# barlettacarmen/CrCNN

Measured on AMD Instinct MI355X. Metric: encrypted images/sec, higher is better.
Workload: dtype u64

## Files before the change

crcnn_amd/binding.py:

```python
import ctypes
import os
import re

import numpy as np

_HERE = os.path.dirname(os.path.abspath(__file__))
LIB_PATH = os.path.join(_HERE, "lib", "libcrcnn_hip.so")
HEADER = os.path.join(os.path.dirname(_HERE), "include", "crcnn_hip.h")

u64 = ctypes.c_uint64
PU = ctypes.POINTER(u64)
VP = ctypes.c_void_p
CI = ctypes.c_int
SZ = ctypes.c_size_t

COEFF, NTT, NTTP, NTTL, NTTL1, NTTLC, NTTLS = 0, 1, 2, 3, 4, 5, 6


class CrcError(RuntimeError):
    def __init__(self, status, what=""):
        self.status = status
        super().__init__(f"{what}: {_strerror(status)} (status {status}, hip error {_lib.crc_last_hip_error() if _lib else '?'})")


# ... 78 lines not shown
    L.crc_square_relin.argtypes = [VP, VP, SZ, VP, CI, VP, VP, VP]
    L.crc_square_relin_forms.argtypes = [VP, VP, CI, SZ, VP, CI, VP, CI, VP, VP]
    L.crc_square_pool_relin_supported.argtypes = [VP, CI, CI, CI]
    L.crc_square_pool_relin_work_bytes.restype = SZ; L.crc_square_pool_relin_work_bytes.argtypes = [VP] + [CI] * 9
    L.crc_square_pool_relin_forms.argtypes = [VP, VP, CI] + [CI] * 8 + [VP, CI, VP, VP, CI, VP, VP]
    L.crc_poly2_relin_work_bytes.restype = SZ; L.crc_poly2_relin_work_bytes.argtypes = [VP, SZ, CI]
    L.crc_poly2_relin_forms.argtypes = [VP, VP, CI, SZ, VP, CI, VP, VP, VP, VP, CI, VP, VP]
    L.crc_multiply_relin_work_bytes.restype = SZ; L.crc_multiply_relin_work_bytes.argtypes = [VP, SZ, CI]
    L.crc_multiply.argtypes = [VP, VP, VP, SZ, VP, VP, VP]
    L.crc_multiply_relin_forms.argtypes = [VP, VP, VP, CI, SZ, VP, CI, VP, CI, VP, VP]
    L.crc_poly3_relin_work_bytes.restype = SZ; L.crc_poly3_relin_work_bytes.argtypes = [VP, SZ, CI]
    L.crc_poly3_relin_forms.argtypes = [VP, VP, CI, SZ, VP, CI, VP, VP, VP, VP, VP, CI, VP, VP]
    L.crc_poly2_pool_relin_supported.argtypes = [VP, CI, CI, CI]
    L.crc_poly2_pool_relin_work_bytes.restype = SZ; L.crc_poly2_pool_relin_work_bytes.argtypes = [VP] + [CI] * 9
    L.crc_poly2_pool_relin_forms.argtypes = [VP, VP, CI] + [CI] * 8 + [VP, CI, VP, VP, VP, VP, CI, VP, VP]
    L.crc_conv2d_forms.argtypes = [VP, VP, VP, CI, VP] + [CI] * 9 + [CI, CI, VP, VP, VP]
    L.crc_dense_forms.argtypes = [VP, VP, VP, CI, VP, CI, CI, CI, CI, CI, VP, VP, VP]
    L.crc_pack28.argtypes = [VP, VP, SZ, CI, VP]
    L.crc_limb_supported.argtypes = [VP, CI, CI, CI]
    L.crc_limb_tensor_bytes.restype = SZ; L.crc_limb_tensor_bytes.argtypes = [VP, CI, CI, CI, CI]
    L.crc_limb_weights_bytes.restype = SZ; L.crc_limb_weights_bytes.argtypes = [VP, CI, CI, CI, CI]
    L.crc_limb_pack_weights.argtypes = [VP, VP, CI, CI, CI, CI, VP, VP]
    L.crc_limb_pack_weights_tile.argtypes = [VP, VP, CI, CI, CI, CI, CI, CI, VP, VP]
    L.crc_limb_pack_tensor_at.argtypes = [VP, VP, CI, CI, CI, CI, CI, VP, CI, CI, VP]
    L.crc_plan_mac.argtypes = [VP] + [CI] * 10 + [ctypes.POINTER(CI)]
    L.crc_plan_mac_scalar.argtypes = [VP] + [CI] * 9 + [ctypes.POINTER(CI)]
    L.crc_scalar_weights_bytes.restype = SZ; L.crc_scalar_weights_bytes.argtypes = [VP, CI, CI, CI, CI]
    L.crc_scalar_supported.argtypes = [VP] + [CI] * 9
    L.crc_scalar_pack_weights.argtypes = [VP, VP, CI, CI, CI, CI, CI, VP, ctypes.POINTER(CI), VP]
    L.crc_plan_fold_pool.argtypes = [VP] + [CI] * 12 + [ctypes.POINTER(CI)]
    L.crc_plan_hoist_pool.argtypes = [VP] + [CI] * 22 + [ctypes.POINTER(CI)]
    L.crc_limb_pack_tensor.argtypes = [VP, VP, CI, CI, CI, CI, CI, VP, VP]
    L.crc_limb_conv1_supported.argtypes = [VP] + [CI] * 8
    L.crc_limb_conv1_weights_bytes.restype = SZ; L.crc_limb_conv1_weights_bytes.argtypes = [VP]
    L.crc_limb_conv1_pack_weights.argtypes = [VP, VP, CI, CI, CI, VP, VP]
    L.crc_limb_conv1_weights_bytes_for.restype = SZ; L.crc_limb_conv1_weights_bytes_for.argtypes = [VP, CI, CI, CI]
    L.crc_limb_conv1_form.argtypes = [VP] + [CI] * 8
    L.crc_conv2d_forms_work_bytes.restype = SZ; L.crc_conv2d_forms_work_bytes.argtypes = [VP] + [CI] * 12
    L.crc_square.argtypes = [VP, VP, SZ, VP, VP, VP]
    L.crc_relinearize.argtypes = [VP, VP, SZ, VP, CI, VP, VP, VP]
    L.crc_import_seal.argtypes = [VP, PU, CI, PU]
    L.crc_export_seal.argtypes = [VP, PU, CI, PU]
    L.crc_params_hash.argtypes = [VP, PU]
    for f_ in ("ct", "evk", "pk", "sk"):
        getattr(L, f"crc_seal_{f_}_bytes").restype = SZ
    L.crc_seal_ct_bytes.argtypes = [VP, CI]; L.crc_seal_evk_bytes.argtypes = [VP, CI]; L.crc_seal_pk_bytes.argtypes = [VP]; L.crc_seal_sk_bytes.argtypes = [VP]
    L.crc_seal_ct_save.argtypes = [VP, PU, CI, VP, SZ, ctypes.POINTER(SZ)]
    L.crc_seal_ct_load.argtypes = [VP, VP, SZ, PU, CI, ctypes.POINTER(CI), ctypes.POINTER(SZ)]
    L.crc_seal_evk_save.argtypes = [VP, PU, CI, VP, SZ, ctypes.POINTER(SZ)]
    L.crc_seal_evk_load.argtypes = [VP, VP, SZ, PU, ctypes.POINTER(CI)]
    L.crc_seal_pk_save.argtypes = [VP, PU, VP, SZ, ctypes.POINTER(SZ)]
    L.crc_seal_pk_load.argtypes = [VP, VP, SZ, PU]
    L.crc_seal_sk_save.argtypes = [VP, PU, VP, SZ, ctypes.POINTER(SZ)]
    L.crc_seal_sk_load.argtypes = [VP, VP, SZ, PU]
    L.crc_h5_dataset_count.argtypes = [ctypes.c_char_p, ctypes.c_char_p, ctypes.POINTER(SZ)]
    L.crc_h5_read_f32.argtypes = [ctypes.c_char_p, ctypes.c_char_p, ctypes.POINTER(ctypes.c_float), SZ, ctypes.POINTER(SZ)]
    L.crc_h5_list.argtypes = [ctypes.c_char_p, ctypes.c_char_p, SZ]
    L.crc_keygen.argtypes = [VP, u64, PU, PU]
    L.crc_gen_evk.argtypes = [VP, u64, PU, CI, PU]
    L.crc_encrypt.argtypes = [VP, PU, PU, SZ, u64, PU]
    L.crc_encrypt_dev_work_bytes.restype = SZ; L.crc_encrypt_dev_work_bytes.argtypes = [VP, SZ]
    L.crc_encrypt_dev.argtypes = [VP, VP, VP, SZ, u64, VP, VP, VP]
    PB = ctypes.POINTER(ctypes.c_uint8)
    L.crc_random_key.argtypes = [PB]
    L.crc_chacha20_block.argtypes = [PB, ctypes.c_uint32, PB, PB]
    L.crc_keygen_key.argtypes = [VP, PB, PU, PU]
# ... 415 lines not shown
                                   self.p(d_y), self.p(d_work), self.stream), "crc_conv2d")
        else:
            _chk(self.L.crc_conv2d_forms(self.c, self.p(d_x), self.p(d_w), w_form, self.p(d_bias), B, zd, xd, yd, xs, ys, xf, yf, nf, in_form, out_form,
                                         self.p(d_y), self.p(d_work), self.stream), "crc_conv2d_forms")

    def limb_supported(self, zd, xf=1, yf=1):
        return bool(self.L.crc_limb_supported(self.c, zd, xf, yf))

    def limb_tensor_bytes(self, B, zd, xd=1, yd=1):
        return self.L.crc_limb_tensor_bytes(self.c, B, zd, xd, yd)

    def limb_weights_bytes(self, nf, zd, xf=1, yf=1):
        return self.L.crc_limb_weights_bytes(self.c, nf, zd, xf, yf)

    def limb_pack_weights(self, d_w_ntt, nf, zd, xf, yf, d_wl):
        _chk(self.L.crc_limb_pack_weights(self.c, self.p(d_w_ntt), nf, zd, xf, yf, self.p(d_wl), self.stream), "crc_limb_pack_weights")

    def plan_mac(self, zd, xd, yd, xs, ys, xf, yf, nf, B, matrix_cores=True):
        wf = CI(0)
        _chk(self.L.crc_plan_mac(self.c, zd, xd, yd, xs, ys, xf, yf, nf, int(B or 0), 1 if matrix_cores else 0, ctypes.byref(wf)), "crc_plan_mac")
        return wf.value

    def plan_fold_pool(self, zd, xd, yd, xs, ys, xf, yf, nf, pxs, pys, pxf, pyf):
        f = CI(0)
        _chk(self.L.crc_plan_fold_pool(self.c, zd, xd, yd, xs, ys, xf, yf, nf, pxs, pys, pxf, pyf, ctypes.byref(f)), "crc_plan_fold_pool")
        return bool(f.value)

    def plan_hoist_pool(self, up, conv, pool, B, matrix_cores=True):
        h = CI(0)
        _chk(self.L.crc_plan_hoist_pool(self.c, *(tuple(up) if up else (0,) * 8), *conv, *pool, int(B or 0), 1 if matrix_cores else 0, ctypes.byref(h)),
             "crc_plan_hoist_pool")
        return bool(h.value)

    def scalar_weights_bytes(self, nf, zd, xf=1, yf=1):
        return self.L.crc_scalar_weights_bytes(self.c, nf, zd, xf, yf)

    def scalar_supported(self, B, zd, xd, yd, xs, ys, xf, yf, nf):
        return bool(self.L.crc_scalar_supported(self.c, B, zd, xd, yd, xs, ys, xf, yf, nf))

    def scalar_pack_weights(self, d_w, w_stride, nf, zd, xf, yf, d_ws):
        const = CI(1)
        rc = self.L.crc_scalar_pack_weights(self.c, self.p(d_w), w_stride, nf, zd, xf, yf, self.p(d_ws), ctypes.byref(const), self.stream)
        if rc == -1 and const.value == 0:
            return False
        _chk(rc, "crc_scalar_pack_weights")
        return True

    def plan_mac_scalar(self, zd, xd, yd, xs, ys, xf, yf, nf, B):
        wf = CI(0)
        _chk(self.L.crc_plan_mac_scalar(self.c, zd, xd, yd, xs, ys, xf, yf, nf, int(B or 0), ctypes.byref(wf)), "crc_plan_mac_scalar")
        return wf.value

    def limb_pack_weights_tile(self, d_w_tile, nf, f0, ft, zd, xf, yf, d_wl):
        _chk(self.L.crc_limb_pack_weights_tile(self.c, self.p(d_w_tile), nf, f0, ft, zd, xf, yf, self.p(d_wl), self.stream), "crc_limb_pack_weights_tile")

    def limb_pack_tensor(self, d_x, in_form, B, zd, xd, yd, d_xl):
        _chk(self.L.crc_limb_pack_tensor(self.c, self.p(d_x), in_form, B, zd, xd, yd, self.p(d_xl), self.stream), "crc_limb_pack_tensor")

    def limb_pack_tensor_at(self, d_x, in_form, B, zd, xd, yd, d_xl, Btot, b0):
        _chk(self.L.crc_limb_pack_tensor_at(self.c, self.p(d_x), in_form, B, zd, xd, yd, self.p(d_xl), Btot, b0, self.stream), "crc_limb_pack_tensor_at")

    def limb_conv1_supported(self, zd, xd, yd, xs, ys, xf, yf, nf):
        return bool(self.L.crc_limb_conv1_supported(self.c, zd, xd, yd, xs, ys, xf, yf, nf))

    def limb_conv1_weights_bytes(self):
        return self.L.crc_limb_conv1_weights_bytes(self.c)
# ... 300 lines not shown
```

crcnn_amd/csrc/abi.hip:

```cpp
#include <cstdlib>
#include <cstring>
#include "kernels.h"
#include "chacha.h"
#include "work_arena.h"

#define CHECK_CTX(c) do { if (!(c) || (c)->device < 0) return CRC_ERR_INVALID_ARGUMENT; \
        int dev_ = -1; if (hipGetDevice(&dev_) != hipSuccess || dev_ != (c)->device) HIPCHK(hipSetDevice((c)->device)); } while (0)
#define RUN(x) do { int rc_ = (x); if (rc_) return rc_; } while (0)
static inline hipStream_t S(void *s) { return (hipStream_t)s; }
static inline bool form_ok(int f) { return f == CRC_COEFF || f == CRC_NTT; }
static inline bool nform_ok(int f) { return f == CRC_COEFF || f == CRC_NTT || f == CRC_NTTP; }
static inline bool lform_ok(int f) { return nform_ok(f) || f == CRC_NTTL; }
static inline bool limb_in(int f) { return f == CRC_NTTL || f == CRC_NTTLS; }
static inline u64 *work_base(void *d_work) { return WorkArena(d_work).take<u64>(0); }
static inline size_t work_bytes(size_t words) { WorkArena a; a.take<u64>(words); return a.bytes(); }

extern "C" int crc_plain_to_ntt(crc_ctx *c, const uint64_t *d_plain, size_t count, uint64_t *d_out, void *stream)
{
    CHECK_CTX(c); if (!d_plain || !d_out) return CRC_ERR_INVALID_ARGUMENT;
    return k_plain_ntt(c, d_plain, count, 1, true, d_out, S(stream));
}
extern "C" int crc_plain_expand(crc_ctx *c, const uint64_t *d_compact, size_t count, uint64_t *d_plain, void *stream)
{
    CHECK_CTX(c); if (!d_compact || !d_plain) return CRC_ERR_INVALID_ARGUMENT;
// ... 101 lines not shown
    if (!crc_limb_supported(c, zd, 1, 1)) return CRC_ERR_UNSUPPORTED;
    return k_limb_pack_tensor(c, d_x, (signed char *)d_xl, B, zd, xd * yd, in_form == CRC_NTTP, S(stream), Btot, b0);
}
extern "C" int crc_limb_conv1_supported(const crc_ctx *c, int zd, int xd, int yd, int xs, int ys, int xf, int yf, int nf)
{
    if (!c || nf < 1 || !conv_shape_ok(xd, yd, xs, ys, xf, yf)) return 0;
    return k_limb_conv1_shape(c, zd, xd, yd, xs, ys, xf, yf, nf) ? 1 : 0;
}
extern "C" size_t crc_limb_conv1_weights_bytes(const crc_ctx *c) { return c ? k_limb_conv1_weights_bytes(c) : 0; }
extern "C" size_t crc_limb_conv1_weights_bytes_for(const crc_ctx *c, int nf, int xf, int yf)
{
    return c && nf >= 1 && xf >= 1 && yf >= 1 ? k_limb_conv1_weights_bytes_for(c, nf, xf, yf) : 0;
}
extern "C" int crc_limb_conv1_form(const crc_ctx *c, int zd, int xd, int yd, int xs, int ys, int xf, int yf, int nf)
{
    return crc_limb_conv1_supported(c, zd, xd, yd, xs, ys, xf, yf, nf) ? k_limb_conv1_form(c, xf, yf, nf) : 0;
}
extern "C" int crc_limb_conv1_pack_weights(crc_ctx *c, const uint64_t *d_w_ntt, int nf, int xf, int yf, void *d_wl, void *stream)
{
    CHECK_CTX(c); if (!d_w_ntt || !d_wl || nf < 1 || nf > 32 || xf < 1 || yf < 1 || xf > 8 || yf > 8) return CRC_ERR_INVALID_ARGUMENT;
    if (!k_limb_supported(c, 64)) return CRC_ERR_UNSUPPORTED;
    return k_limb_conv1_pack_weights(c, d_w_ntt, (signed char *)d_wl, nf, xf, yf, S(stream));
}
static int conv1_sub_batch(const crc_ctx *c, int B, int xd, int yd, int xf, int yf, int nf, int P, int out_form)
{
    if (out_form == CRC_NTTL || B <= 1) return B;
    const size_t per = k_limb_conv1_image_bytes(c, 1, xd, yd, xf, yf, nf) + (out_form == CRC_NTTLC ? 0 : 8 * k_limb_result_words(c, 1, nf, P));
    const long long ev = c->tune.conv1_pass_bytes;
    const size_t cap = ev > 0 ? (size_t)ev : (size_t)16 << 30;
    const size_t fit = cap / (per ? per : 1);
    return (int)(fit < 1 ? 1 : fit > (size_t)B ? (size_t)B : fit);
}
struct Limb1Work { signed char *Xr; u64 *Ys, *buf; int Bs, out_form; };
static Limb1Work limb1_layout(const crc_ctx *c, int B, int xd, int yd, int xf, int yf, int nf, int P, int in_form, int out_form, WorkArena &a)
{
    Limb1Work L{};
    L.out_form = out_form == CRC_NTTLC && P == 1 ? CRC_NTTL : out_form;
    L.Bs = conv1_sub_batch(c, B, xd, yd, xf, yf, nf, P, L.out_form);
    L.Xr = a.take<signed char>(k_limb_conv1_image_bytes(c, L.Bs, xd, yd, xf, yf, nf));
    if (L.out_form != CRC_NTTLC) L.Ys = a.take<u64>(k_limb_result_words(c, L.Bs, nf, P));
    if (in_form == CRC_COEFF) L.buf = a.take<u64>((size_t)L.Bs * xd * yd * crc_ct_words(c, 2));
    return L;
}
static int conv2d_limb1(crc_ctx *c, const uint64_t *d_x, const void *d_wl, const uint64_t *d_bias, int B, int xd, int yd, int xs, int ys, int xf, int yf,
    int nf,
                        int in_form, int out_form, uint64_t *d_y, void *d_work, hipStream_t st)
{
    const int xo = (xd - xf) / xs + 1, yo = (yd - yf) / ys + 1, P = xo * yo, in_cts = xd * yd;
    WorkArena a(d_work);
    const Limb1Work L = limb1_layout(c, B, xd, yd, xf, yf, nf, P, in_form, out_form, a);
    out_form = L.out_form;
    const size_t ctw = crc_ct_words(c, 2);
    for (int b0 = 0; b0 < B; b0 += L.Bs) {
        const int Bn = B - b0 < L.Bs ? B - b0 : L.Bs;
        const u64 *xn = d_x + (size_t)b0 * in_cts * ctw; bool packed = in_form == CRC_NTTP;
        if (in_form == CRC_COEFF) { RUN(k_ntt_ct(c, false, xn, L.buf, (size_t)Bn * in_cts, 2, false, st, nullptr, 0, 0, 0, 0)); xn = L.buf; packed = false; }
        RUN(k_limb_conv1(c, xn, packed, L.Xr, (const signed char *)d_wl, L.Ys, out_form == CRC_NTTLC ? (signed char *)d_y : nullptr, B, b0,
            out_form != CRC_COEFF ? d_bias : nullptr,
                         Bn, xd, yd, xs, ys, xf, yf, nf, st));
        if (out_form == CRC_NTTLC) continue;
        if (out_form == CRC_NTTL) return k_limb_result_to_limb(c, L.Ys, (signed char *)d_y, B, nf * P, st);
        RUN(k_limb_result_to_rows(c, L.Ys, d_y + (size_t)b0 * nf * P * ctw, (size_t)Bn * nf * P * 2, out_form == CRC_NTTP, st));
    }
    if (out_form == CRC_COEFF) RUN(k_ntt_ct(c, true, d_y, d_y, (size_t)B * nf * P, 2, false, st, d_bias, 1, (size_t)P, nf));
    return CRC_OK;
}
struct LimbWork { u64 *Ys; signed char *Xl; u64 *buf; };
static LimbWork limb_layout(const crc_ctx *c, int B, int zd, int xd, int yd, int nf, int P, int in_form, WorkArena &a)
{
    LimbWork L{};
    L.Ys = a.take<u64>(k_limb_result_words(c, B, nf, P));
    if (!limb_in(in_form)) L.Xl = a.take<signed char>(k_limb_tensor_bytes(c, B, zd, xd * yd));
    if (in_form == CRC_COEFF) L.buf = a.take<u64>((size_t)B * zd * xd * yd * crc_ct_words(c, 2));
    return L;
}
extern "C" size_t crc_conv2d_forms_work_bytes(const crc_ctx *c, int B, int zd, int xd, int yd, int xs, int ys, int xf, int yf, int nf, int in_form,
    int w_form, int out_form)
{
    if (!c || !conv_shape_ok(xd, yd, xs, ys, xf, yf)) return 0;
    const int P = ((xd - xf) / xs + 1) * ((yd - yf) / ys + 1);
    WorkArena a;
    if (w_form == CRC_NTTL1) limb1_layout(c, B, xd, yd, xf, yf, nf, P, in_form, out_form, a);
    else if (w_form == CRC_NTTL || w_form == CRC_NTTLS) limb_layout(c, B, zd, xd, yd, nf, P, in_form, a);
    else conv_layout(c, B, zd, xd, yd, xf, yf, P, in_form, a);
    return a.bytes();
}
extern "C" size_t crc_conv2d_work_bytes(const crc_ctx *c, int B, int zd, int xd, int yd, int xs, int ys, int xf, int yf, int nf, int in_form)
{
    return crc_conv2d_forms_work_bytes(c, B, zd, xd, yd, xs, ys, xf, yf, nf, in_form, CRC_NTT, CRC_COEFF);
}
static int conv2d_limb(crc_ctx *c, const uint64_t *d_x, const void *d_wl, const uint64_t *d_bias, int B, int zd, int xd, int yd, int xs, int ys, int xf,
    int yf, int nf,
                       int in_form, int out_form, uint64_t *d_y, void *d_work, hipStream_t st, bool scalar = false)
{
    if (!(scalar ? k_scalar_supported(c, B, zd, xd, yd, xs, ys, xf, yf, nf) : crc_limb_supported(c, zd, xf, yf) != 0)) return CRC_ERR_UNSUPPORTED;
    const int xo = (xd - xf) / xs + 1, yo = (yd - yf) / ys + 1, P = xo * yo, in_cts = zd * xd * yd;
    WorkArena a(d_work);
    const LimbWork L = limb_layout(c, B, zd, xd, yd, nf, P, in_form, a);
    const signed char *xl = (const signed char *)d_x;
    if (!limb_in(in_form)) {
        const u64 *xn = d_x; bool packed = in_form == CRC_NTTP;
        if (in_form == CRC_COEFF) { RUN(k_ntt_ct(c, false, d_x, L.buf, (size_t)B * in_cts, 2, false, st, nullptr, 0, 0, 0, 0)); xn = L.buf; packed = false; }
        RUN(k_limb_pack_tensor(c, xn, L.Xl, B, zd, xd * yd, packed, st, 0, 0, scalar));
        xl = L.Xl;
    }
    if (out_form == (scalar ? CRC_NTTLS : CRC_NTTL) && k_limb_direct_dense(P))
        return k_limb_mac(c, xl, (const signed char *)d_wl, L.Ys, (signed char *)d_y, d_bias, B, zd, xd, yd, xs, ys, xf, yf, nf, st, scalar);
    RUN(k_limb_mac(c, xl, (const signed char *)d_wl, L.Ys, nullptr, out_form != CRC_COEFF ? d_bias : nullptr, B, zd, xd, yd, xs, ys, xf, yf, nf, st, scalar));
    if (limb_in(out_form)) return k_limb_result_to_limb(c, L.Ys, (signed char *)d_y, B, nf * P, st, out_form == CRC_NTTLS);
    RUN(k_limb_result_to_rows(c, L.Ys, d_y, (size_t)B * nf * P * 2, out_form == CRC_NTTP, st));
    if (out_form == CRC_COEFF) RUN(k_ntt_ct(c, true, d_y, d_y, (size_t)B * nf * P, 2, false, st, d_bias, 1, (size_t)P, nf));
    return CRC_OK;
}

extern "C" int crc_conv2d_forms(crc_ctx *c, const uint64_t *d_x, const uint64_t *d_w, int w_form, const uint64_t *d_bias, int B, int zd, int xd, int yd,
// ... 14 lines not shown
        if (B == 0) return CRC_OK;
        return conv2d_limb(c, d_x, d_w, d_bias, B, zd, xd, yd, xs, ys, xf, yf, nf, in_form, out_form, d_y, d_work, S(stream));
    }
    if (w_form == CRC_NTTLS) {
        const bool in_ok = nform_ok(in_form) || (xd * yd == 1 ? in_form == CRC_NTTLS : in_form == CRC_NTTL);
        if (!d_x || !d_w || !d_y || !d_work || B < 0 || zd < 1 || nf < 1 || !(lform_ok(out_form) || out_form == CRC_NTTLS) || !conv_shape_ok(xd, yd, xs, ys, xf,
            yf) || !in_ok) return CRC_ERR_INVALID_ARGUMENT;
        if (B == 0) return CRC_OK;
        return conv2d_limb(c, d_x, d_w, d_bias, B, zd, xd, yd, xs, ys, xf, yf, nf, in_form, out_form, d_y, d_work, S(stream), true);
    }
    if (!d_x || !d_w || !d_y || !d_work || B < 0 || zd < 1 || nf < 1 || !nform_ok(in_form) || !nform_ok(out_form) || (w_form != CRC_NTT && w_form != CRC_NTTP))
        return CRC_ERR_INVALID_ARGUMENT;
    if (!conv_shape_ok(xd, yd, xs, ys, xf, yf)) return CRC_ERR_INVALID_ARGUMENT;
    if (B == 0) return CRC_OK;
    const int xo = (xd - xf) / xs + 1, yo = (yd - yf) / ys + 1, P = xo * yo, T = zd * xf * yf, in_cts = zd * xd * yd;
    hipStream_t st = S(stream);
    WorkArena a(d_work);
    const ConvWork L = conv_layout(c, B, zd, xd, yd, xf, yf, P, in_form, a);
    RUN(k_conv_offsets(c, L.xoff, L.toff, L.toffw, P, T, in_cts, xd, yd, xs, ys, xf, yf, yo, st));
    const u64 *xn = d_x;
    int xp = in_form == CRC_NTTP;
    if (in_form == CRC_COEFF) {
        int maxbits = 0; for (int i = 0; i < c->k; i++) if ((int)c->tabs[i].m.bits > maxbits) maxbits = c->tabs[i].m.bits;
        xp = maxbits <= 55;
        RUN(k_ntt_ct(c, false, d_x, L.buf, (size_t)B * in_cts, 2, false, st, nullptr, 0, 0, 0, xp));
        xn = L.buf;
    }
    RUN(k_mac2(c, xn, d_w, d_y, L.xoff, L.toff, B, P, nf, T, in_cts, out_form != CRC_COEFF ? d_bias : nullptr, xd, yd, xf, yf, L.toffw, st, xp, w_form == CRC_NTTP,
        out_form == CRC_NTTP));
    if (out_form == CRC_COEFF)
        RUN(k_ntt_ct(c, true, d_y, d_y, (size_t)B * nf * P, 2, false, st, d_bias, 1, (size_t)P, nf));
    return CRC_OK;
}
extern "C" int crc_conv2d(crc_ctx *c, const uint64_t *d_x, const uint64_t *d_w, const uint64_t *d_bias, int B, int zd, int xd, int yd,
                          int xs, int ys, int xf, int yf, int nf, int in_form, int out_form, uint64_t *d_y, void *d_work, void *stream)
{
    if (!form_ok(in_form) || !form_ok(out_form)) return CRC_ERR_INVALID_ARGUMENT;
    return crc_conv2d_forms(c, d_x, d_w, CRC_NTT, d_bias, B, zd, xd, yd, xs, ys, xf, yf, nf, in_form, out_form, d_y, d_work, stream);
}
extern "C" int crc_dense_forms(crc_ctx *c, const uint64_t *d_x, const uint64_t *d_w, int w_form, const uint64_t *d_bias, int B, int in_dim, int out_dim,
                               int in_form, int out_form, uint64_t *d_y, void *d_work, void *stream)
{
    return crc_conv2d_forms(c, d_x, d_w, w_form, d_bias, B, in_dim, 1, 1, 1, 1, 1, 1, out_dim, in_form, out_form, d_y, d_work, stream);
}
extern "C" int crc_pack28(crc_ctx *c, uint64_t *d_rows, size_t rows, int unpack, void *stream)
{
    CHECK_CTX(c); if (!d_rows) return CRC_ERR_INVALID_ARGUMENT;
    return k_pack28(c, d_rows, rows, unpack != 0, S(stream));
}

extern "C" size_t crc_dense_work_bytes(const crc_ctx *c, int B, int in_dim, int out_dim, int in_form)
{
    return crc_conv2d_work_bytes(c, B, in_dim, 1, 1, 1, 1, 1, 1, out_dim, in_form);
}
extern "C" int crc_dense(crc_ctx *c, const uint64_t *d_x, const uint64_t *d_w, const uint64_t *d_bias, int B, int in_dim, int out_dim,
                         int in_form, int out_form, uint64_t *d_y, void *d_work, void *stream)
{
    return crc_conv2d(c, d_x, d_w, d_bias, B, in_dim, 1, 1, 1, 1, 1, 1, out_dim, in_form, out_form, d_y, d_work, stream);
}

extern "C" int crc_conv2d_fold_pool(crc_ctx *c, const uint64_t *d_w, const uint64_t *d_bias_ntt, const uint64_t *d_div_ntt, int nf, int zd, int xf, int yf,
                                    int cxs, int cys, int pxf, int pyf, uint64_t *d_w_out, uint64_t *d_bias_out, void *stream)
{
    CHECK_CTX(c);
    if (!d_w || !d_bias_ntt || !d_w_out || !d_bias_out || nf < 1 || zd < 1 || xf < 1 || yf < 1 || cxs < 1 || cys < 1 || pxf < 1 ||
        pyf < 1) return CRC_ERR_INVALID_ARGUMENT;
// ... 86 lines not shown
    CHECK_CTX(c);
    if (!d_w || !d_ws || !constant || nf < 1 || zd < 1 || xf < 1 || yf < 1 || (w_stride != 1 && w_stride != c->n)) return CRC_ERR_INVALID_ARGUMENT;
    if (c->k > 8 || !k_limb_supported(c, k_limb_steps(zd, xf, yf) * 32)) return CRC_ERR_UNSUPPORTED;
    return k_scalar_pack_weights(c, d_w, (size_t)w_stride, (signed char *)d_ws, nf, zd, xf, yf, constant, S(stream));
}
extern "C" int crc_plan_mac_scalar(const crc_ctx *c, int zd, int xd, int yd, int xs, int ys, int xf, int yf, int nf, int B, int *w_form)
{
    RUN(crc_plan_mac(c, zd, xd, yd, xs, ys, xf, yf, nf, B, 1, w_form));
    if (c->tune.scalar_mac && zd >= 2 && k_scalar_supported(c, B < 1 ? 1 : B, zd, xd, yd, xs, ys, xf, yf, nf)) *w_form = CRC_NTTLS;
    return CRC_OK;
}
extern "C" int crc_plan_fold_pool(const crc_ctx *c, int zd, int xd, int yd, int xs, int ys, int xf, int yf, int nf, int pxs, int pys, int pxf, int pyf,
    int *fold)
{
    if (!c || !fold || zd < 1 || nf < 1 || !conv_shape_ok(xd, yd, xs, ys, xf, yf) || pxs < 1 || pys < 1 || pxf < 1 || pyf < 1) return CRC_ERR_INVALID_ARGUMENT;
    *fold = 0;
    const int xo = (xd - xf) / xs + 1, yo = (yd - yf) / ys + 1;
    const int xf2 = (pxf - 1) * xs + xf, yf2 = (pyf - 1) * ys + yf, xs2 = xs * pxs, ys2 = ys * pys;
    if (xf2 > xd || yf2 > yd || pxf > xo || pyf > yo) return CRC_OK;
    const int xo2 = (xd - xf2) / xs2 + 1, yo2 = (yd - yf2) / ys2 + 1;
    if (xo2 != (xo - pxf) / pxs + 1 || yo2 != (yo - pyf) / pys + 1) return CRC_OK;
    const long long fpad = (nf + 7) / 8 * 8, T1 = (long long)zd * xf * yf, T2 = (long long)zd * xf2 * yf2;
    const long long cost_sep = fpad * xo * yo * (T1 + 24) + (long long)nf * xo2 * yo2 * 10 * (pxf * pyf + 1);
    const long long cost_fused = fpad * xo2 * yo2 * (T2 + 24);
    *fold = cost_fused < cost_sep ? 1 : 0;
    return CRC_OK;
}

static long long plan_mac_cost(const crc_ctx *c, int zd, int xd, int yd, int xs, int ys, int xf, int yf, int nf, int B, int matrix_cores)
{
    int wf = CRC_NTT;
    if (crc_plan_mac(c, zd, xd, yd, xs, ys, xf, yf, nf, B, matrix_cores, &wf) != CRC_OK) return -1;
    const long long P = (long long)((xd - xf) / xs + 1) * ((yd - yf) / ys + 1);
    if (wf == CRC_NTTL1) return 32 * ((2 * P + 15) / 16 * 8) * ((k_limb_conv1_form(c, xf, yf, nf) == 2 ? 40 : 64) + 24) * 25 / 16;
    if (wf == CRC_NTTL) return (long long)(nf + 31) / 32 * 32 * P * ((long long)k_limb_steps(zd, xf, yf) * 32 + 24);
    return (long long)(nf + 7) / 8 * 8 * P * ((long long)zd * xf * yf + 24);
}
extern "C" int crc_plan_hoist_pool(const crc_ctx *c, int uzd, int uxd, int uyd, int uxs, int uys, int uxf, int uyf, int unf, int zd, int xd, int yd, int xs,
                                   int ys, int xf, int yf, int nf, int pxs, int pys, int pxf, int pyf, int B, int matrix_cores, int *hoist)
{
    if (!c || !hoist || zd < 1 || nf < 1 || !conv_shape_ok(xd, yd, xs, ys, xf, yf) || pxs < 1 || pys < 1 || pxf < 1 || pyf < 1) return CRC_ERR_INVALID_ARGUMENT;
    *hoist = 0;
    if (!c->tune.hoist_pool || xs != 1 || ys != 1 || pxs * pys == 1) return CRC_OK;
    int fold = 0;
    { const int rc = crc_plan_fold_pool(c, zd, xd, yd, xs, ys, xf, yf, nf, pxs, pys, pxf, pyf, &fold); if (rc != CRC_OK) return rc; }
    if (!fold) return CRC_OK;
    if (uzd < 1 || unf != zd || !conv_shape_ok(uxd, uyd, uxs, uys, uxf, uyf) || (uxd - uxf) / uxs + 1 != xd || (uyd - uyf) / uys + 1 != yd) return CRC_OK;
    const int uxf2 = (pxf - 1) * uxs + uxf, uyf2 = (pyf - 1) * uys + uyf, sxd = xd - pxf + 1, syd = yd - pyf + 1;
    if (uxf2 > uxd || uyf2 > uyd || !conv_shape_ok(uxd, uyd, uxs, uys, uxf2, uyf2)) return CRC_OK;
    if ((uxd - uxf2) / uxs + 1 != sxd || (uyd - uyf2) / uys + 1 != syd) return CRC_OK;
    const int xo = xd - xf + 1, yo = yd - yf + 1;
    if (!conv_shape_ok(sxd, syd, pxs, pys, xf, yf) || (sxd - xf) / pxs + 1 != (xo - pxf) / pxs + 1 || (syd - yf) / pys + 1 != (yo - pyf) / pys + 1) return CRC_OK;
    int uf = CRC_NTT, uf2 = CRC_NTT;
    if (crc_plan_mac(c, uzd, uxd, uyd, uxs, uys, uxf, uyf, unf, B, matrix_cores, &uf) != CRC_OK) return CRC_OK;
    if (crc_plan_mac(c, uzd, uxd, uyd, uxs, uys, uxf2, uyf2, unf, B, matrix_cores, &uf2) != CRC_OK) return CRC_OK;
    if ((uf == CRC_NTTL1 || uf == CRC_NTTL) && uf2 != uf) return CRC_OK;
    const int xf2 = xf + pxf - 1, yf2 = yf + pyf - 1;
    const long long folded = plan_mac_cost(c, uzd, uxd, uyd, uxs, uys, uxf, uyf, unf, B, matrix_cores) +
                             plan_mac_cost(c, zd, xd, yd, pxs, pys, xf2, yf2, nf, B, matrix_cores);
    const long long hoisted = plan_mac_cost(c, uzd, uxd, uyd, uxs, uys, uxf2, uyf2, unf, B, matrix_cores) +
                              plan_mac_cost(c, zd, sxd, syd, pxs, pys, xf, yf, nf, B, matrix_cores);
    *hoist = hoisted < folded ? 1 : 0;
    return CRC_OK;
}

static size_t square_chunk(const crc_ctx *c)
{
    if (c->tune.sq_chunk > 0) return (size_t)c->tune.sq_chunk;
    const size_t nk = (size_t)c->n * c->k;
    return nk <= 32768 ? 1024 : nk <= 65536 ? 512 : nk <= 131072 ? 256 : 128;
}

struct ActWork { u64 *xh, *s, *kp, *y3, *rest; size_t step; };
enum { ACT_XH = 1, ACT_S = 2, ACT_MULTIPLY = 4 };
static ActWork act_layout(const crc_ctx *c, size_t planes, size_t pin, size_t pout, int dbc, int regions, WorkArena &a)
{
    ActWork L{};
    L.step = square_chunk(c) / pin ? square_chunk(c) / pin : 1;
    const size_t pp = planes < L.step ? planes : L.step, cin = pp * pin, cout = pp * pout;
    const size_t pr = regions & ACT_MULTIPLY ? k_multiply_work_words(c, cin) : k_square_work_words(c, cin), rl = k_relin_work_words(c, cout, dbc);
    if (regions & ACT_XH) L.xh = a.take<u64>(cin * crc_ct_words(c, 2));
    if (regions & ACT_S) L.s = a.take<u64>(cin * crc_ct_words(c, 2));
    L.kp = a.take<u64>(k_relin_keys_words(c, dbc));
    L.y3 = a.take<u64>(cin * crc_ct_words(c, 3));
    L.rest = a.take<u64>(pr > rl ? pr : rl);
    return L;
}
static size_t act_bytes(const crc_ctx *c, size_t planes, size_t pin, size_t pout, int dbc, int regions)
{
    WorkArena a;
    act_layout(c, planes, pin, pout, dbc, regions, a);
    return a.bytes();
}
static inline size_t pass_len(size_t count, size_t o, size_t step) { return count - o < step ? count - o : step; }
static int ntt_copy(crc_ctx *c, const u64 *x, size_t ch, u64 *xh, void *stream)
{
    HIPCHK(hipMemcpyAsync(xh, x, 8 * ch * crc_ct_words(c, 2), hipMemcpyDeviceToDevice, S(stream)));
    return crc_ntt_fwd(c, xh, ch, 2, stream);
// ... 503 lines not shown
```

crcnn_amd/csrc/ctx.cpp:

```cpp
#include "ctx.h"
#include "host_parallel.h"
#include <algorithm>
#include <cstring>
#include <cstdlib>
#include <string>

typedef unsigned __int128 u128;

static thread_local int g_last_hip = 0;
int crc_set_hip_error(hipError_t e) { g_last_hip = (int)e; return CRC_ERR_HIP; }

extern "C" int crc_last_hip_error(void) { return g_last_hip; }
extern "C" int crc_version(void) { return 100; }
extern "C" const char *crc_strerror(int s)
{
    switch (s) {
    case CRC_OK: return "ok";
    case CRC_ERR_INVALID_ARGUMENT: return "invalid argument";
    case CRC_ERR_PARAMETERS: return "encryption parameters are not set correctly";
    case CRC_ERR_HIP: return "HIP runtime error";
    case CRC_ERR_UNSUPPORTED: return "unsupported parameter combination";
    case CRC_ERR_IO: return "I/O error";
    case CRC_ERR_NOT_FOUND: return "not found";
    case CRC_ERR_COMM: return "RCCL error";
// ... 108 lines not shown
                u64 u = a[j], v = a[j + t];
                u64 s = addmod(u, v, q);
                a[j] = (s & 1) ? (u64)(((u128)s + q) >> 1) : s >> 1;
                a[j + t] = h_mulmod(submod(u, v, q), w, q);
            }
        }
    }
}

static const u64 kAuxMods[] = {
    0x1fffffffffb40001ULL, 0x1fffffffff500001ULL, 0x1fffffffff380001ULL, 0x1fffffffff000001ULL, 0x1ffffffffef00001ULL,
    0x1ffffffffee80001ULL, 0x1ffffffffeb40001ULL, 0x1ffffffffe780001ULL, 0x1ffffffffe600001ULL, 0x1ffffffffe4c0001ULL };
static const u64 kMsk = 0x1fffffffffe00001ULL, kMtilde = 1ULL << 32, kGamma = 0x1fffffffffc80001ULL;

static u64 prod_mod(const u64 *v, int cnt, int skip, u64 m)
{
    u64 r = 1 % m;
    for (int j = 0; j < cnt; j++) if (j != skip) r = h_mulmod(r, v[j] % m, m);
    return r;
}

static void read_tuning(CrcTuning &t)
{
    auto geti = [](const char *name, long long dflt) { const char *e = getenv(name); return e && *e ? atoll(e) : dflt; };
    t.no_fold = getenv("CRC_NO_FOLD") ? 1 : 0;
    t.ntt_inv61_loose = getenv("CRC_NTT_INV61_LOOSE") ? 1 : 0;
    t.mfma_order = (int)geti("CRC_MFMA_ORDER", -1);
    t.mfma_variant = (int)geti("CRC_MFMA_VARIANT", 2);
    { const int v = (int)geti("CRC_MFMA_RING", 0); t.mfma_ring = v >= 3 && v <= 5 ? v : 0; }
    { const int v = (int)geti("CRC_CONV1_WAVES", 0); t.conv1_waves = v == 8 || v == 12 ? v : 0; }
    t.conv1_narrow = (int)geti("CRC_CONV1_NARROW", 1);
    { const int v = (int)geti("CRC_CONV1_FORM", 0); t.conv1_form = v == 1 || v == 2 ? v : 0; }
    t.hoist_pool = geti("CRC_HOIST_POOL", 1) ? 1 : 0;
    { const long long v = geti("CRC_CONV1_PASS_BYTES", 0); t.conv1_pass_bytes = v > 0 ? v : 0; }
    { const int v = (int)geti("CRC_LIMB_PACK_GROUP", 1); t.limb_pack_group = v > 0 ? v : 1; }
    t.mac2_cfg = (int)geti("CRC_MAC2_CFG", 0);
    t.mac_order = (int)geti("CRC_MAC_ORDER", -1);
    t.mac_regstage = (int)geti("CRC_MAC_REGSTAGE", 0);
    t.mac_stream = (int)geti("CRC_MAC_STREAM", 1);
    t.mac2_dbg = (int)geti("CRC_MAC2_DBG", 0);
    t.relin_path = (int)geti("CRC_RELIN_PATH", 0);
    t.sq_path = (int)geti("CRC_SQ_PATH", 0);
    t.sq_chunk = (int)geti("CRC_SQ_CHUNK", 0);
    t.sq_fuse = (int)geti("CRC_SQ_FUSE", -1);
    t.f64_radix = (int)geti("CRC_F64_RADIX", 0);
    t.f64_wave = (int)geti("CRC_F64_WAVE", -1);
    t.ntt_wave = (int)geti("CRC_NTT_WAVE", -1);
    t.mfma_min_steps = (int)geti("CRC_MFMA_MIN_STEPS", 0);
    t.scalar_mac = geti("CRC_SCALAR_MAC", 1) ? 1 : 0;
    t.relin_mac_ct = (int)geti("CRC_RELIN_MAC_CT", 0);
    t.ntt_split = (int)geti("CRC_NTT_SPLIT", 1);
    t.poly_tail = (int)geti("CRC_POLY_TAIL", 0);
}
extern "C" int crc_ctx_set_tuning(crc_ctx *c, const char *name, long long value)
{
    if (!c || !name) return CRC_ERR_INVALID_ARGUMENT;
    const std::string s(name);
    CrcTuning &t = c->tune;
    if (s == "mfma_order") t.mfma_order = (int)value;
    else if (s == "mfma_variant") t.mfma_variant = (int)value;
    else if (s == "mfma_ring") t.mfma_ring = value >= 3 && value <= 5 ? (int)value : 0;
    else if (s == "conv1_waves") t.conv1_waves = value == 8 || value == 12 ? (int)value : 0;
    else if (s == "conv1_narrow") t.conv1_narrow = (int)value;
    else if (s == "conv1_form") t.conv1_form = value == 1 || value == 2 ? (int)value : 0;
    else if (s == "hoist_pool") t.hoist_pool = value ? 1 : 0;
    else if (s == "conv1_pass_bytes") t.conv1_pass_bytes = value > 0 ? value : 0;
    else if (s == "limb_pack_group") t.limb_pack_group = value > 0 ? (int)value : 1;
    else if (s == "mac2_cfg") t.mac2_cfg = (int)value;
    else if (s == "mac_order") t.mac_order = (int)value;
    else if (s == "mac_regstage") t.mac_regstage = (int)value;
    else if (s == "mac_stream") t.mac_stream = (int)value;
    else if (s == "ntt_inv61_loose") t.ntt_inv61_loose = value ? 1 : 0;
    else if (s == "relin_path") t.relin_path = (int)value;
    else if (s == "sq_path") t.sq_path = (int)value;
    else if (s == "sq_chunk") t.sq_chunk = (int)value;
    else if (s == "sq_fuse") t.sq_fuse = (int)value;
    else if (s == "f64_radix") t.f64_radix = (int)value;
    else if (s == "f64_wave") t.f64_wave = (int)value;
    else if (s == "ntt_wave") t.ntt_wave = (int)value;
    else if (s == "mfma_min_steps") t.mfma_min_steps = (int)value;
    else if (s == "scalar_mac") t.scalar_mac = value ? 1 : 0;
    else if (s == "relin_mac_ct") t.relin_mac_ct = (int)value;
    else if (s == "ntt_split") t.ntt_split = (int)value;
    else if (s == "poly_tail") t.poly_tail = value ? 1 : 0;
    else return CRC_ERR_NOT_FOUND;
    return CRC_OK;
}

extern "C" int crc_default_coeff_modulus_128(int n, uint64_t *q, int cap)
{
    static const u64 m1024[] = {0x7e00001}, m2048[] = {0x3fffffff000001}, m4096[] = {0x7fffffff380001, 0x3fffffff000001},
        m8192[] = {0x7fffffff380001, 0x7ffffffef00001, 0x3fffffff000001, 0x3ffffffef40001},
        m16384[] = {0x7fffffff380001, 0x7ffffffef00001, 0x7ffffffeac0001, 0x7ffffffe700001, 0x7ffffffe600001, 0x7ffffffe4c0001, 0x3fffffff000001,
            0x3ffffffef40001};
    const u64 *src; int cnt;
    switch (n) {
    case 1024: src = m1024; cnt = 1; break;
    case 2048: src = m2048; cnt = 1; break;
// ... 417 lines not shown
```

crcnn_amd/csrc/ctx.h:

```cpp
#pragma once
#include <hip/hip_runtime.h>
#include <atomic>
#include <mutex>
#include <unordered_map>
#include <vector>
#include "modarith.h"
#include "f64mod.h"
#include "../../include/crcnn_hip.h"

#define CRC_MAXK 8
#define CRC_MAXB (CRC_MAXK + 2)

struct PlainParams {
    u64 threshold;
    u64 inc[CRC_MAXK];
    int fast;
    u64 delta[CRC_MAXK];
    u64 uhi[CRC_MAXK];
};

struct BehzParams {
    int k, ka, kb;
    u64 t;
    u64 m_tilde, m_sk;
// ... 30 lines not shown
    u64 p0_mod_q[CRC_MAXK];
};

#define CRC_NF64A 12
struct Sq64Params {
    int kf;
    F64Mod m[CRC_NF64A];
    double lift_c[CRC_NF64A][CRC_MAXK][4];
    double lift_r[CRC_NF64A][2];
    double floor_x[CRC_NF64A][2];
    double floor_c[CRC_NF64A][CRC_MAXK][4];
    double inv_mhat[CRC_NF64A][2];
    double mhat_msk[CRC_NF64A][2];
    double inv_B_msk[2];
    u64 mhat_q[CRC_MAXK][CRC_NF64A];
    u64 B_q[CRC_MAXK];
};

struct HostNtt {
    ModParams m;
    u64 root, inv_n;
    std::vector<u64> rp, srp, irp2, sirp2;
    std::vector<u64> irp, sirp;
};

struct CrcTuning {
    int no_fold = 0;
    int ntt_inv61_loose = 0;
    int mfma_order = -1;
    int mfma_variant = 2;
    int mfma_ring = 0;
    int conv1_waves = 0;
    int conv1_narrow = 1;
    int hoist_pool = 1;
    int conv1_form = 0;
    long long conv1_pass_bytes = 0;
    int limb_pack_group = 1;
    int mac2_cfg = 0;
    int mac_order = -1;
    int mac_regstage = 0;
    int mac_stream = 1;
    int mac2_dbg = 0;
    int ntt_split = 1;
    int relin_mac_ct = 0;
    int scalar_mac = 1;
    int mfma_min_steps = 0;
    int f64_radix = 0;
    int sq_chunk = 0;
    int sq_fuse = -1;
    int ntt_wave = -1;
    int f64_wave = -1;
    int sq_path = 0;
    int poly_tail = 0;
    int relin_path = 0;
};

struct SlotTables {
    HostNtt T;
    std::vector<u32> idx;
    u64 one_s = 0;
    bool lazy = false;
    ulonglong2 *d_fwd = nullptr, *d_inv = nullptr;
    u32 *d_idx = nullptr;
};

struct crc_ctx {
// ... 45 lines not shown
```

crcnn_amd/csrc/kernels.h:

```cpp
#pragma once
#include "ctx.h"

static inline unsigned xcd_grid(size_t groups, unsigned G) { return (unsigned)((groups + 7) / 8 * 8 * G); }

int k_ntt_ct(crc_ctx *c, bool inv, const u64 *src, u64 *dst, size_t count, int size, bool bsk, hipStream_t st,
             const u64 *addend, int add_sign, size_t add_group, int add_mod = 0, int pack_out = 0);
int k_ntt_ct_fwd_mul(crc_ctx *c, u64 *ct, size_t count, const u64 *w, size_t group, hipStream_t st);
int k_ntt_ct_fwd_fma(crc_ctx *c, u64 *ct, size_t count, const u64 *u, const u64 *key, hipStream_t st);
int k_ntt_ct_fwd_negmul(crc_ctx *c, u64 *ct, size_t count, const u64 *sk, hipStream_t st);
int k_ntt_ct_poly0(crc_ctx *c, const u64 *src, u64 *dst, size_t count, hipStream_t st);
int k_ntt_ct_addct(crc_ctx *c, const u64 *src, u64 *dst, size_t count, const u64 *addct, int add_size, hipStream_t st);
int k_ntt_ct_head_add(crc_ctx *c, const u64 *src, int src_size, u64 *dst, size_t count, const u64 *addrows, hipStream_t st);
int k_spread_ntt(crc_ctx *c, const u64 *src, size_t items, u64 *dst, hipStream_t st);
int k_digit_ntt(crc_ctx *c, const u64 *src, int src_size, int src_poly, size_t count, int D, const unsigned char *dig_i, const unsigned char *dig_shift, int dbc,
                u64 *dst, hipStream_t st, int pack_out = 0);
int k_square_intt(crc_ctx *c, const u64 *src, u64 *dst, size_t count, bool bsk, hipStream_t st, const u64 *opt_mul = nullptr, bool *applied = nullptr);
int k_multiply_intt(crc_ctx *c, const u64 *x, const u64 *y, u64 *dst, size_t count, bool bsk, hipStream_t st, const u64 *opt_mul = nullptr, bool *applied = nullptr);
int k_ntt_ct_inv_scaled(crc_ctx *c, const u64 *src, u64 *dst, size_t count, int size, const u64 *mul, const u64 *mul_s, hipStream_t st);
int k_plain_ntt(crc_ctx *c, const u64 *d_plain, size_t count, int mode, bool do_ntt, u64 *d_out, hipStream_t st);
int k_plain_expand(crc_ctx *c, const u64 *d_compact, size_t count, u64 *d_plain, hipStream_t st);
int k_rowwise(crc_ctx *c, u64 *acc, const u64 *b, size_t count, int size, int op, int sign, size_t group, size_t gmod, hipStream_t st);
int k_pool(crc_ctx *c, const u64 *x, u64 *y, int B, int zd, int xd, int yd, int xs, int ys, int xf, int yf, const u64 *mul, hipStream_t st, int pack_out = 0);
int k_pad(crc_ctx *c, const u64 *x, u64 *y, int B, int zd, int xd, int yd, int px0, int px1, int py0, int py1, hipStream_t st);
int k_bn_ntt(crc_ctx *c, u64 *x, int B, int zd, int hw, const u64 *mean, const u64 *invstd, hipStream_t st);
// ... 49 lines not shown
int k_noise_budget(crc_ctx *c, const u64 *sk, const u64 *ct, size_t cnt, int size, bool in_ntt, int32_t *bits, int32_t *min_out, u64 *work, hipStream_t st);
int k_budget_bits_host(const crc_ctx *c, const u64 *h_v, size_t cnt, int32_t *h_bits);

int k_slots_compose(crc_ctx *c, const long long *d_values, size_t count, int slots, size_t item_stride, size_t slot_stride, u64 *d_plain, hipStream_t st);
int k_slots_decompose(crc_ctx *c, const u64 *d_plain, size_t count, int slots, long long *d_values, size_t item_stride, size_t slot_stride, hipStream_t st);
int k_slots_compose_host(crc_ctx *c, const long long *values, size_t count, int slots, size_t item_stride, size_t slot_stride, u64 *plain);
int k_slots_decompose_host(crc_ctx *c, const u64 *plain, size_t count, int slots, long long *values, size_t item_stride, size_t slot_stride);
int k_slots_rescale(crc_ctx *c, const u64 *d_in, size_t count, u64 divisor, u64 *d_out, hipStream_t st);
int k_slots_rescale_host(crc_ctx *c, const u64 *plain_in, size_t count, u64 divisor, u64 *plain_out);

bool   k_limb_supported(const crc_ctx *c, int T);
size_t k_limb_tensor_bytes(const crc_ctx *c, int B, int zd, int npos);
size_t k_limb_weights_bytes(const crc_ctx *c, int nf, int zd, int xf, int yf);
int    k_limb_flat_zdc(int zd);
int    k_limb_steps(int zd, int xf, int yf);
size_t k_limb_result_words(const crc_ctx *c, int B, int nf, int P);
int k_limb_pack_tensor(crc_ctx *c, const u64 *x, signed char *xl, int B, int zd, int npos, bool packed, hipStream_t st, int Btot = 0, int b0 = 0, bool scalar = false);
int k_limb_pack_weights(crc_ctx *c, const u64 *w, signed char *wl, int nf, int zd, int xf, int yf, hipStream_t st, int f0 = 0, int ft = -1);
int k_limb_result_to_rows(crc_ctx *c, const u64 *ys, u64 *y, size_t rows, bool pack_out, hipStream_t st);
int k_limb_result_to_limb(crc_ctx *c, const u64 *ys, signed char *xl, int B, int zd, hipStream_t st, bool scalar = false);
bool k_limb_direct_dense(int P);
int k_limb_mac(crc_ctx *c, const signed char *xl, const signed char *wl, u64 *ys, signed char *xl_out, const u64 *bias_ntt, int B, int zd, int xd, int yd, int xs, int ys_, int xf, int yf, int nf,
               hipStream_t st, bool scalar = false);
size_t k_scalar_weights_bytes(const crc_ctx *c, int nf, int zd, int xf, int yf);
bool   k_scalar_supported(const crc_ctx *c, int B, int zd, int xd, int yd, int xs, int ys_, int xf, int yf, int nf);
int k_scalar_pack_weights(crc_ctx *c, const u64 *w, size_t wstride, signed char *wl, int nf, int zd, int xf, int yf, int *constant, hipStream_t st);
bool   k_limb_conv1_shape(const crc_ctx *c, int zd, int xd, int yd, int xs, int ys_, int xf, int yf, int nf);
int    k_limb_conv1_form(const crc_ctx *c, int xf, int yf, int nf);
size_t k_limb_conv1_weights_bytes(const crc_ctx *c);
size_t k_limb_conv1_weights_bytes_for(const crc_ctx *c, int nf, int xf, int yf);
size_t k_limb_conv1_image_bytes(const crc_ctx *c, int B, int xd, int yd, int xf, int yf, int nf);
int k_limb_conv1_pack_weights(crc_ctx *c, const u64 *w, signed char *wl, int nf, int xf, int yf, hipStream_t st);
int k_limb_conv1(crc_ctx *c, const u64 *x, bool packed, signed char *xr, const signed char *wl, u64 *ys, signed char *xl_out, int Bout, int b0, const u64 *bias_ntt, int B, int xd, int yd,
                 int xs, int ys_, int xf, int yf, int nf, hipStream_t st);
```

crcnn_amd/csrc/kernels_mfma1.hip:

```cpp
#include "kernels.h"
#include "limbred.h"
#include <cstdlib>

typedef int v4i __attribute__((ext_vector_type(4)));
typedef signed char i8;
#define NPL 7
#define MAXK 8

struct Conv1Args {
    const i8 *xr; const i8 *wl; u64 *ys; i8 *xl_out; const ModParams *mods; const u64 *bias;
    int n, k, B, Bout, b0, xd, yo, xs, ystr, P, F, mtiles;
    unsigned img_stride, plane_bytes, poly_bytes;
    unsigned out_img_bytes;
    int out_zdc;
    int narrow;
    int acc0[MAXK][13];
    u32 qbits[MAXK], qfold[MAXK];
    unsigned px_rs;
    int px_taps, px_yf, px_pair;
    int acc7[MAXK][7];
};

__device__ __forceinline__ void limb_digits1(u64 r, u64 q, int (&d)[NPL])
{
// ... 297 lines not shown
    const u64 q = mods[i].q;
    const int lane = threadIdx.x & (RSL - 1), qrow = (threadIdx.x >> 5) & (RG - 1), h = threadIdx.x >> 7, row = rg * RG + qrow;
    {
        u32 pl[NPL][4];
#pragma unroll
        for (int l = 0; l < NPL; l++)
#pragma unroll
            for (int wv = 0; wv < 4; wv++) pl[l][wv] = 0;
        if (row < xd) {
            const u64 *src = x + ((((size_t)b * xd * yd + (size_t)row * yd + h * 16) * 2 + c) * k + i) * (size_t)n + s0 + lane;
#pragma unroll
            for (int colx = 0; colx < 16; colx++)
                if (h * 16 + colx < yd) {
                    u64 v = src[(size_t)colx * 2 * k * n];
                    if (packed) v = (v & 0xffffffffULL) | ((v >> 32) << 28);
                    const u64 dg = balanced_digit_bytes(v, q);
#pragma unroll
                    for (int l = 0; l < NPL; l++) pl[l][colx >> 2] |= (u32)((dg >> (8 * l)) & 0xff) << (8 * (colx & 3));
                }
        }
        i8 *sp = st + (size_t)lane * (NPL * RG * 32) + qrow * 32 + h * 16;
#pragma unroll
        for (int l = 0; l < NPL; l++) *reinterpret_cast<uint4 *>(sp + l * (RG * 32)) = make_uint4(pl[l][0], pl[l][1], pl[l][2], pl[l][3]);
    }
    __syncthreads();
    const int pieces_per_run = RG * 2, rows_here = min(RG, xd - rg * RG);
    for (int o = threadIdx.x; o < RSL * NPL * pieces_per_run; o += 256) {
        const int run = o / pieces_per_run, part = o - run * pieces_per_run, sl = run / NPL, l = run - sl * NPL;
        if ((part >> 1) >= rows_here) continue;
        i8 *dst = xr + (((size_t)i * n + s0 + sl) * B + b) * img_stride + (size_t)l * plane_bytes + (size_t)c * poly_bytes + (size_t)(rg * RG) * 32 + part * 16;
        *reinterpret_cast<uint4 *>(dst) = *reinterpret_cast<const uint4 *>(st + (size_t)run * (RG * 32) + part * 16);
    }
}
__global__ void __launch_bounds__(256) limb_pack_rows1_kernel_px(const u64 *x, i8 *xr, const ModParams *mods, int n, int k, int B, int xd, int yd, int packed,
                                                                 unsigned img_stride, unsigned poly_bytes, unsigned rs)
{
    extern __shared__ __attribute__((aligned(16))) i8 stp[];
    const unsigned sstride = RG * rs + 16;
    const int sblocks = n / RSL;
    const int sb = blockIdx.x % (sblocks * k), i = sb / sblocks, s0 = (sb % sblocks) * RSL;
    const int rgs = (xd + RG - 1) / RG;
    size_t r = blockIdx.x / (sblocks * k);
    const int rg = (int)(r % rgs); r /= rgs; const int c = (int)(r % 2); const int b = (int)(r / 2);
    const u64 q = mods[i].q;
    const int lane = threadIdx.x & (RSL - 1), qrow = (threadIdx.x >> 5) & (RG - 1), h = threadIdx.x >> 7, row = rg * RG + qrow;
    if (row < xd) {
        const u64 *src = x + ((((size_t)b * xd * yd + (size_t)row * yd + h * 16) * 2 + c) * k + i) * (size_t)n + s0 + lane;
        u64 *sp = reinterpret_cast<u64 *>(stp + (size_t)lane * sstride + qrow * rs) + h * 16;
#pragma unroll
        for (int colx = 0; colx < 16; colx++) {
            const int col = h * 16 + colx;
            if ((unsigned)col * 8 >= rs) continue;
            u64 dg = 0;
            if (col < yd) {
                u64 v = src[(size_t)colx * 2 * k * n];
                if (packed) v = (v & 0xffffffffULL) | ((v >> 32) << 28);
                dg = balanced_digit_bytes(v, q);
            }
            sp[colx] = dg;
        }
    }
    __syncthreads();
    const int per_run = RG * rs / 16, valid = min(RG, xd - rg * RG) * (int)rs / 16;
    for (int o = threadIdx.x; o < RSL * per_run; o += 256) {
        const int sl = o / per_run, part = o - sl * per_run;
        if (part >= valid) continue;
        i8 *dst = xr + (((size_t)i * n + s0 + sl) * B + b) * img_stride + (size_t)c * poly_bytes + (size_t)(rg * RG) * rs + part * 16;
        *reinterpret_cast<uint4 *>(dst) = *reinterpret_cast<const uint4 *>(stp + (size_t)sl * sstride + part * 16);
    }
}
__global__ void __launch_bounds__(64) limb_pack_w1_kernel(const u64 *w, i8 *wl, const ModParams *mods, int n, int k, int F, int xf, int yf)
{
    const int sblocks = n / 64;
    const int sb = blockIdx.x % (sblocks * k), i = sb / sblocks, s = (sb % sblocks) * 64 + threadIdx.x;
    size_t r = blockIdx.x / (sblocks * k);
    const int ky = (int)(r % yf); r /= yf; const int kx = (int)(r % xf); const int f = (int)(r / xf);
    const ModParams m = mods[i];
    int d[NPL]; limb_digits1(w[((((size_t)f * xf + kx) * yf + ky) * k + i) * (size_t)n + s], m.q, d);
    i8 *dst = wl + ((size_t)i * n + s) * (NPL * 32 * 64) + f * 64 + kx * 8 + ky;
#pragma unroll
    for (int l = 0; l < NPL; l++) dst[(size_t)l * (32 * 64)] = (i8)d[l];
}

__global__ void __launch_bounds__(64) limb_pack_w1_kernel_px(const u64 *w, i8 *wl, const ModParams *mods, int n, int k, int F, int xf, int yf)
{
    const int sblocks = n / 64;
    const int sb = blockIdx.x % (sblocks * k), i = sb / sblocks, s = (sb % sblocks) * 64 + threadIdx.x;
    size_t r = blockIdx.x / (sblocks * k);
    const int ky = (int)(r % yf); r /= yf; const int kx = (int)(r % xf); const int f = (int)(r / xf);
    const ModParams m = mods[i];
    u64 v = w[((((size_t)f * xf + kx) * yf + ky) * k + i) * (size_t)n + s];
    const int tap = kx * yf + ky, G = tap >> 1;
    i8 *dst = wl + ((size_t)i * n + s) * (NPL * NJ * 32 * 64) + ((G >> 2) * 32 + f) * 64 + (G & 3) * 16 + (tap & 1) * 8;
    for (int l = 0; l < NPL; l++) {
        int d[NPL]; limb_digits1(v, m.q, d);
#pragma unroll
        for (int dm = 0; dm < NPL; dm++) dst[(size_t)dm * (NJ * 32 * 64) + l] = (i8)d[dm];
        v = mulmod(v, 256, m);
    }
}

static inline unsigned conv1_poly_bytes(int xd) { return ((unsigned)xd + 1) * 32; }
static inline unsigned conv1_img_stride(int xd) { const unsigned b = NPL * 2 * conv1_poly_bytes(xd); return (b + 1023) / 1024 * 1024; }
static inline unsigned conv1_px_rs(int yd) { return ((unsigned)yd * 8 + 15) / 16 * 16; }
static inline unsigned conv1_px_poly_bytes(int xd, int yd) { const unsigned b = (unsigned)xd * conv1_px_rs(yd); return b + (128 + 256 - b % 256) % 256; }
static inline unsigned conv1_px_img_stride(int xd, int yd) { return (2 * conv1_px_poly_bytes(xd, yd) + 1023) / 1024 * 1024; }
static bool conv1_fits(unsigned img_stride, int xd, int yd, int xs, int ys_, int xf, int yf)
{
    const int xo = (xd - xf) / xs + 1, yo = (yd - yf) / ys_ + 1;
    return 2 * (size_t)img_stride + (size_t)NPL * xo * yo * 2 * 32 <= 160 * 1024;
}
int k_limb_conv1_form(const crc_ctx *c, int xf, int yf, int nf)
{
    bool px = xf * yf <= 8 * NJ;
    for (int i = 0; i < c->k && px; i++) px = conv1_fold7_ok(c->tabs[i].m.q, c->tabs[i].m.bits, fold_constant(c->tabs[i].m.q, c->tabs[i].m.bits));
    const int forced = c->tune.conv1_form;
    if (forced == 1 || !px) return 1;
    if (forced == 2) return 2;
    return nf > 16 && nf <= 20 ? 1 : 2;
}
bool k_limb_conv1_shape(const crc_ctx *c, int zd, int xd, int yd, int xs, int ys_, int xf, int yf, int nf)
{
    if (zd != 1 || xf > 8 || yf > 8 || nf > 32 || yd > 32 || c->n < 64 || c->k > MAXK) return false;
    for (int i = 0; i < c->k; i++) if (!conv1_fold_ok(c->tabs[i].m.q, c->tabs[i].m.bits, fold_constant(c->tabs[i].m.q, c->tabs[i].m.bits))) return false;
    const int xo = (xd - xf) / xs + 1, yo = (yd - yf) / ys_ + 1;
    if (xo * yo > 1024) return false;
    return conv1_fits(k_limb_conv1_form(c, xf, yf, nf) == 2 ? conv1_px_img_stride(xd, yd) : conv1_img_stride(xd), xd, yd, xs, ys_, xf, yf);
}
static size_t conv1_form_weights_bytes(const crc_ctx *c, int form) { return (size_t)c->n * c->k * NPL * 32 * 64 * (form == 2 ? NJ : 1); }
size_t k_limb_conv1_weights_bytes(const crc_ctx *c) { return conv1_form_weights_bytes(c, 2); }
size_t k_limb_conv1_weights_bytes_for(const crc_ctx *c, int nf, int xf, int yf) { return conv1_form_weights_bytes(c, k_limb_conv1_form(c, xf, yf, nf)); }
size_t k_limb_conv1_image_bytes(const crc_ctx *c, int B, int xd, int yd, int xf, int yf, int nf)
{
    return (size_t)c->n * c->k * B * (k_limb_conv1_form(c, xf, yf, nf) == 2 ? conv1_px_img_stride(xd, yd) : conv1_img_stride(xd));
}

static void conv1_tables(const crc_ctx *c, Conv1Args &a)
{
    for (int i = 0; i < c->k; i++) { conv1_bias_table(c->tabs[i].m.q, a.acc0[i]); conv1_bias7_table(c->tabs[i].m.q, a.acc7[i]); a.qbits[i] = c->tabs[i].m.bits;
        a.qfold[i] = fold_constant(c->tabs[i].m.q, c->tabs[i].m.bits); }
}

int k_limb_conv1_pack_weights(crc_ctx *c, const u64 *w, i8 *wl, int nf, int xf, int yf, hipStream_t st)
{
    const int form = k_limb_conv1_form(c, xf, yf, nf);
    HIPCHK(hipMemsetAsync(wl, 0, conv1_form_weights_bytes(c, form), st));
    const size_t blocks = (size_t)(c->n / 64) * c->k * nf * xf * yf;
    if (form == 2) hipLaunchKernelGGL(limb_pack_w1_kernel_px, dim3((unsigned)blocks), dim3(64), 0, st, w, wl, c->d_mods, c->n, c->k, nf, xf, yf);
    else hipLaunchKernelGGL(limb_pack_w1_kernel, dim3((unsigned)blocks), dim3(64), 0, st, w, wl, c->d_mods, c->n, c->k, nf, xf, yf);
    HIPCHK(hipGetLastError());
    return CRC_OK;
}
int k_limb_conv1(crc_ctx *c, const u64 *x, bool packed, i8 *xr, const i8 *wl, u64 *ys, i8 *xl_out, int Bout, int b0, const u64 *bias_ntt, int B, int xd,
    int yd, int xs, int ys_,
                 int xf, int yf, int nf, hipStream_t st)
{
    if (B == 0) return CRC_OK;
    if (!k_limb_conv1_shape(c, 1, xd, yd, xs, ys_, xf, yf, nf)) return CRC_ERR_UNSUPPORTED;
    const int xo = (xd - xf) / xs + 1, yo = (yd - yf) / ys_ + 1;
    const int form = k_limb_conv1_form(c, xf, yf, nf);
    Conv1Args a{};
    a.xr = xr; a.wl = wl; a.ys = ys; a.xl_out = xl_out; a.mods = c->d_mods; a.bias = bias_ntt;
    a.n = c->n; a.k = c->k; a.B = B; a.Bout = Bout; a.b0 = b0; a.xd = xd; a.yo = yo; a.xs = xs; a.ystr = ys_; a.P = xo * yo; a.F = nf;
        a.mtiles = (2 * a.P + 15) / 16;
    a.out_zdc = a.P > 1 ? k_limb_flat_zdc(nf) : 0;
    a.out_img_bytes = a.out_zdc ? (unsigned)((NPL * 2 * a.P * a.out_zdc + 15) / 16 * 16) : (unsigned)(NPL * a.P * 2 * 32);
    conv1_tables(c, a);
    const size_t pack_blocks = (size_t)(c->n / RSL) * c->k * B * 2 * ((xd + RG - 1) / RG);
    if (pack_blocks > 0x7fffffffULL) return CRC_ERR_INVALID_ARGUMENT;
    if (form == 2) {
        a.px_rs = conv1_px_rs(yd); a.poly_bytes = conv1_px_poly_bytes(xd, yd); a.img_stride = conv1_px_img_stride(xd, yd);
        a.px_taps = xf * yf; a.px_yf = yf;
        a.px_pair = yf % 2 == 0 && ys_ % 2 == 0 ? 1 : 0;
        hipLaunchKernelGGL(limb_pack_rows1_kernel_px, dim3((unsigned)pack_blocks), dim3(256), RSL * (RG * a.px_rs + 16), st, x, xr, c->d_mods, c->n, c->k, B, xd,
            yd, packed ? 1 : 0, a.img_stride, a.poly_bytes, a.px_rs);
        HIPCHK(hipGetLastError());
        const size_t lds = 2 * (size_t)a.img_stride + (xl_out ? a.out_img_bytes : 0);
        { const int rc = crc_ctx_ensure_lds(c, (const void *)mfma_conv1_kernel_px, lds); if (rc) return rc; }
        hipLaunchKernelGGL(mfma_conv1_kernel_px, dim3((unsigned)(c->n * c->k)), dim3(64 * 8), lds, st, a);
        HIPCHK(hipGetLastError());
        return CRC_OK;
    }
    a.poly_bytes = conv1_poly_bytes(xd); a.plane_bytes = 2 * a.poly_bytes; a.img_stride = conv1_img_stride(xd);
    a.narrow = c->tune.conv1_narrow != 0 && nf > 16 && nf <= 20 ? 1 : 0;
    {
        hipLaunchKernelGGL(limb_pack_rows1_kernel, dim3((unsigned)pack_blocks), dim3(256), 0, st, x, xr, c->d_mods, c->n, c->k, B, xd, yd, packed ? 1 : 0,
            a.img_stride, a.plane_bytes,
                           a.poly_bytes);
        HIPCHK(hipGetLastError());
    }
    auto busiest = [&](int nw) {
        int load[4] = {0, 0, 0, 0}, worst = 0;
        for (int w = 0; w < nw; w++) load[w & 3] += (a.mtiles - (w >> 1) + nw / 2 - 1) / (nw / 2);
        for (int sd = 0; sd < 4; sd++) worst = load[sd] > worst ? load[sd] : worst;
        return worst;
    };
    const int forced = c->tune.conv1_waves;
    const int nwaves = forced ? forced : a.narrow ? 12 : busiest(12) <= busiest(8) ? 12 : 8;
    const size_t lds = 2 * (size_t)a.img_stride + (xl_out ? a.out_img_bytes : 0);
    { const int rc = crc_ctx_ensure_lds(c, (const void *)mfma_conv1_kernel, lds); if (rc) return rc; }
    hipLaunchKernelGGL(mfma_conv1_kernel, dim3((unsigned)(c->n * c->k)), dim3(64 * nwaves), lds, st, a);
    HIPCHK(hipGetLastError());
    return CRC_OK;
}
```

crcnn_amd/csrc/limbred.h:

```cpp
#pragma once
#include "modarith.h"

CRC_HD u32 crc_alignbit(u32 hi, u32 lo, u32 sh)
{
#if defined(__HIP_DEVICE_COMPILE__)
    return __builtin_amdgcn_alignbit(hi, lo, sh);
#else
    return (u32)((((u64)hi << 32) | lo) >> sh);
#endif
}

CRC_HD u64 diag_reduce(const int (&D)[13], const ModParams &m, u64 qinv)
{
    typedef unsigned __int128 u128;
    const u128 s0 = ((u128)(((u64)(u32)D[12] << 32) | (u32)D[8]) << 64) | (((u64)(u32)D[4] << 32) | (u32)D[0]);
    const u128 s1 = ((u128)(u32)D[9] << 64) | (((u64)(u32)D[5] << 32) | (u32)D[1]);
    const u128 s2 = ((u128)(u32)D[10] << 64) | (((u64)(u32)D[6] << 32) | (u32)D[2]);
    const u128 s3 = ((u128)(u32)D[11] << 64) | (((u64)(u32)D[7] << 32) | (u32)D[3]);
    const u128 U = s0 + (s1 << 8) + (s2 << 16) + (s3 << 24);
    const u64 ulo = (u64)U, uhi = (u64)(U >> 64);
    const u64 mq = ulo * qinv;
    const u64 t = uhi - mulhi64(mq, m.q) + m.q;
    if (m.fold) {
        const u64 r = (t & (((u64)1 << m.bits) - 1)) + (u64)(u32)(t >> m.bits) * (u32)m.fold;
// ... 97 lines not shown
    for (int j = 0; j < 3; j++) P[j] = (u32)E[2 * j] + ((u32)E[2 * j + 1] << 8);
    P[3] = (u32)E[6];
    if (PB) for (int j = 0; j < 4; j++) P[j] += PB[j];
    const u32 o0 = P[1] << 16, o1 = crc_alignbit(P[3], P[1], 16), o2 = P[3] >> 16;
    const u64 ev = ((u64)P[2] << 32) | P[0];
    const u64 lo64 = ev + (((u64)o1 << 32) | o0);
    u[0] = (u32)lo64; u[1] = (u32)(lo64 >> 32); u[2] = o2 + (lo64 < ev);
}
CRC_HD long long fold7_words_centred(u32 u0, u32 u1, u32 u2, u64 q, u32 bits, u32 fold, long long bias_centred)
{
    const u32 sb = bits - 32, m1 = (1u << sb) - 1;
    const u32 uh = crc_alignbit(u2, u1, sb);
    const u64 r = (u64)uh * fold + (((u64)(u1 & m1) << 32) | u0);
    long long t = (long long)(r - q) + bias_centred;
    const long long h = (long long)(q >> 1);
    t += t < -h ? (long long)q : 0;
    t -= t > h ? (long long)q : 0;
    return t;
}
CRC_HD long long diag7_fold_centred(const int (&E)[7], u64 q, u32 bits, u32 fold, long long bias_centred, const u32 *PB = nullptr)
{
    u32 u[3];
    diag7_pack_words(E, PB, u);
    return fold7_words_centred(u[0], u[1], u[2], q, bits, fold, bias_centred);
}
CRC_HD u64 centred_digit_bytes(long long cv) { return ((u64)cv + 0x0080808080808080ULL) ^ 0x0080808080808080ULL; }

CRC_HD u64 balanced_digit_bytes(u64 r, u64 q)
{
    const long long cv = r > (q >> 1) ? (long long)(r - q) : (long long)r;
    return ((u64)cv + 0x0080808080808080ULL) ^ 0x0080808080808080ULL;
}

inline u64 inverse_mod_2_64(u64 q) { u64 inv = q; for (int it = 0; it < 6; it++) inv *= 2 - q * inv; return inv; }

inline void bias_to_multiple(u64 q, long long (&B)[13])
{
    typedef unsigned __int128 u128;
    u128 K0 = 0;
    for (int d = 0; d < 13; d++) K0 += (u128)(u64)B[d] << (8 * d);
    const u64 rem = (u64)(K0 % q);
    long long delta = rem > q / 2 ? (long long)(q - rem) : -(long long)rem;
    for (int d = 0; d < 8 && delta; d++) { const long long dg = (long long)(signed char)(delta & 0xff); B[d] += dg; delta = (delta - dg) >> 8; }
}
inline void limb_bias_table(u64 q, int T, int (&out)[13])
{
    long long B[13];
    for (int d = 0; d < 13; d++) {
        const u64 bound = (u64)T * (u64)((d < 12 - d ? d : 12 - d) + 1) * 16384 + 256;
        u64 b = 1; while (b < bound) b <<= 1;
        B[d] = (long long)b;
    }
    bias_to_multiple(q, B);
    for (int d = 0; d < 13; d++) out[d] = (int)(u32)(u64)B[d];
}
inline void conv1_bias_table(u64 q, int (&out)[13])
{
    long long B[13];
    for (int d = 0; d < 13; d++) B[d] = d <= 10 ? 1 << 23 : d == 11 ? 1 << 21 : 1 << 19;
    bias_to_multiple(q, B);
    for (int d = 0; d < 13; d++) out[d] = (int)B[d];
}

inline void conv1_bias7_table(u64 q, int (&out)[7])
{
    typedef unsigned __int128 u128;
// ... 22 lines not shown
```

crcnn_amd/host/crcnn_host.cpp:

```cpp
#include "crcnn_host.h"
#include "../csrc/host_parallel.h"
#include <algorithm>
#include <atomic>
#include <chrono>
#include <cmath>
#include <cstdlib>
#include <cstring>
#include <fstream>
#include <iostream>
#include <list>
#include <mutex>
#include <sstream>

using namespace std;

crc_ctx *context = nullptr;
static void *g_stream = nullptr;
void setStream(void *s) { g_stream = s; }
void *getStream() { return g_stream; }
static inline void *stream() { return g_stream; }
vector<uint64_t> secret_key, public_key, ev_keys16_host;
shared_ptr<DeviceBuffer> ev_keys16;
static bool g_det = false;
static uint64_t g_det_seed = 0;
// ... 758 lines not shown
    DeviceBuffer fake, outc, wk;
    vector<uint64_t> corr, q;
    BnFold(BatchNormLayer &bn, int T, int per_ch, int max_rows) : bn(bn), T(T), per_ch(per_ch), fake((size_t)T * 2 * K() * N() * 8),
        outc((size_t)max_rows * 2 * K() * N() * 8), wk(max<size_t>(crc_dense_work_bytes(ctx(), 1, T, max_rows, CRC_NTT), 256)),
        corr((size_t)max_rows * 2 * K() * N()), q(K())
    {
        const size_t rowb = (size_t)K() * N() * 8;
        chk(crc_memset(ctx(), fake.ptr, 0, fake.bytes, stream()), "crc_memset");
        for (int z = 0; z < T / per_ch; z++) for (int t = 0; t < per_ch; t++)
            chk(crc_memcpy_d2d(ctx(), (char *)fake.ptr + ((size_t)z * per_ch + t) * 2 * rowb, (char *)bn.d_mean[1]->ptr + (size_t)z * rowb, rowb, stream()),
                "crc_memcpy_d2d");
        chk(crc_ctx_table(ctx(), "q", q.data(), K()) < 0 ? CRC_ERR_INVALID_ARGUMENT : CRC_OK, "crc_ctx_table");
    }
    void apply(uint64_t *d_w, int fn, uint64_t *bias)
    {
        const int n = N(), k = K();
        for (int f = 0; f < fn; f++)
            chk(crc_multiply_plain_ntt(ctx(), d_w + (size_t)f * T * k * n, (const uint64_t *)bn.d_invstd->ptr, T, per_ch, 1, stream()),
                "crc_multiply_plain_ntt");
        chk(crc_dense(ctx(), (const uint64_t *)fake.ptr, d_w, nullptr, 1, T, fn, CRC_NTT, CRC_NTT, (uint64_t *)outc.ptr, wk.ptr, stream()), "crc_dense");
        chk(crc_memcpy_d2h(ctx(), corr.data(), outc.ptr, (size_t)fn * 2 * k * n * 8, stream()), "crc_memcpy_d2h");
        chk(crc_stream_sync(ctx(), stream()), "crc_stream_sync");
        for (int f = 0; f < fn; f++) for (int m = 0; m < k; m++) for (int s2 = 0; s2 < n; s2++) {
            uint64_t &b = bias[((size_t)f * k + m) * n + s2]; const uint64_t c = corr[(((size_t)f * 2) * k + m) * n + s2];
            b = b >= c ? b - c : b + q[m] - c;
        }
    }
};

static bool g_matrix_cores = true;
int MacLayer::plannedForm(int B) const
{
    int wf = CRC_NTT;
    if (slot_weights && g_matrix_cores) chk(crc_plan_mac_scalar(ctx(), zd, xd, yd, xs, ys, xf, yf, nf, B, &wf), "crc_plan_mac_scalar");
    else chk(crc_plan_mac(ctx(), zd, xd, yd, xs, ys, xf, yf, nf, B, g_matrix_cores ? 1 : 0, &wf), "crc_plan_mac");
    return wf;
}
bool MacLayer::limbFits() const
{
    size_t free_b = 0, total_b = 0;
    chk(crc_mem_info(ctx(), &free_b, &total_b), "crc_mem_info");
    return free_b >= crc_limb_weights_bytes(ctx(), nf, zd, xf, yf) + ((size_t)24 << 30);
}
void MacLayer::upload()
{
    if (alreadyNtt()) return;
    vector<const Plaintext *> w, b;
    plaintexts(0, nf, w, &b);
    streamed = forced_placement >= 0 ? forced_placement == 1 : tooLargeForHbm(w.size());
    if (forced_placement >= 0) tilewise = forcedTilewise();
    else if (dense && !streamed && plannedForm(g_expected_batch) == CRC_NTTL) {
        size_t free_b = 0, total_b = 0;
        chk(crc_mem_info(ctx(), &free_b, &total_b), "crc_mem_info");
        const size_t canon = w.size() * (size_t)K() * N() * 8, limb = crc_limb_weights_bytes(ctx(), nf, zd, xf, yf), reserve = (size_t)24 << 30;
        tilewise = (canon + limb + reserve > free_b && limb + reserve + ((size_t)8 << 30) <= free_b) || getenv("CRC_FORCE_TILEWISE") != nullptr;
    }
    if (streamed) d_plain = uploadPlain(w, 3); else if (!tilewise) d_w = uploadPlain(w, 0);
    d_b[0] = uploadPlain(b, 1); d_b[1] = uploadPlain(b, 2);
    alreadyNtt() = true;
}
vector<uint64_t> MacLayer::hostBias()
{
    vector<uint64_t> bias((size_t)nf * K() * N());
    chk(crc_memcpy_d2h(ctx(), bias.data(), d_b[1]->ptr, bias.size() * 8, stream()), "crc_memcpy_d2h");
    chk(crc_stream_sync(ctx(), stream()), "crc_stream_sync");
    return bias;
}
void MacLayer::setBias(const vector<uint64_t> &ntt_rows)
{
// ... 55 lines not shown
        if (!hasPlaintexts()) throw logic_error("FullyConnectedLayer " + name +
            ": tile-wise weights are built on every rank -- a receiving rank must load the model too");
    } else if (allocate_only && !alreadyNtt()) {
        const size_t rowb = (size_t)K() * N() * 8;
        streamed = forced_placement >= 0 ? forced_placement == 1 : tooLargeForHbm(nf * taps());
        if (!streamed) d_w = make_shared<DeviceBuffer>(nf * taps() * rowb);
        d_b[0] = make_shared<DeviceBuffer>(nf * rowb); d_b[1] = make_shared<DeviceBuffer>(nf * rowb);
        alreadyNtt() = true;
    }
    upload();
    if (tilewise) { buildTilewise(); return; }
    packWeights(true);
    if (streamed && !d_plain) d_plain = make_shared<DeviceBuffer>(nf * taps() * N() * 8);
    out.push_back(streamed ? d_plain : d_w); out.push_back(d_b[0]); out.push_back(d_b[1]);
}
bool MacLayer::limbWeights(int B)
{
    upload();
    if (streamed) return false;
    if (tilewise) { buildTilewise(); return true; }
    if (w_form == CRC_NTTL || w_form == CRC_NTTL1 || w_form == CRC_NTTLS) return true;
    int planned = plannedForm(B);
    if (planned == CRC_NTTLS) {
        if (w_form == CRC_NTTP) packWeights(true);
        auto ws = make_shared<DeviceBuffer>(crc_scalar_weights_bytes(ctx(), nf, zd, xf, yf));
        int constant = 1;
        const int rc = crc_scalar_pack_weights(ctx(), (const uint64_t *)d_w->ptr, N(), nf, zd, xf, yf, ws->ptr, &constant, stream());
        if (rc == CRC_OK) { d_w = ws; w_form = CRC_NTTLS; return true; }
        if (constant) chk(rc, "crc_scalar_pack_weights");
        slot_weights = false;
        planned = plannedForm(B);
    }
    const bool conv1 = !dense && planned == CRC_NTTL1;
    if (!conv1 && !(planned == CRC_NTTL && limbFits())) return false;
    if (w_form == CRC_NTTP) packWeights(true);
    auto wl = make_shared<DeviceBuffer>(conv1 ? crc_limb_conv1_weights_bytes_for(ctx(), nf, xf, yf) : crc_limb_weights_bytes(ctx(), nf, zd, xf, yf));
    if (conv1) chk(crc_limb_conv1_pack_weights(ctx(), (const uint64_t *)d_w->ptr, nf, xf, yf, wl->ptr, stream()), "crc_limb_conv1_pack_weights");
    else chk(crc_limb_pack_weights(ctx(), (const uint64_t *)d_w->ptr, nf, zd, xf, yf, wl->ptr, stream()), "crc_limb_pack_weights");
    chk(crc_stream_sync(ctx(), stream()), "crc_stream_sync");
    if (conv1) d_w_canon = d_w;
    d_w = wl; w_form = conv1 ? CRC_NTTL1 : CRC_NTTL;
    return true;
}
void MacLayer::packWeights(bool unpack)
{
    upload();
    if (streamed || (tilewise && !tile_built)) return;
    if (w_form == CRC_NTTL1 && unpack) { d_w = d_w_canon; d_w_canon.reset(); w_form = CRC_NTT; return; }
    if (w_form == CRC_NTTL || w_form == CRC_NTTL1 || w_form == CRC_NTTLS) { if (unpack) throw logic_error(kind() + (" " + name) +
        ": weights are in limb form (fuse() / broadcastParameters() must precede the first forward())"); return; }
    if ((w_form == CRC_NTTP) == !unpack) return;
    chk(crc_pack28(ctx(), (uint64_t *)d_w->ptr, nf * taps() * K(), unpack ? 1 : 0, stream()), "crc_pack28");
    w_form = unpack ? CRC_NTT : CRC_NTTP;
}
ciphertext3D MacLayer::run(const ciphertext3D &input, int zo, int xo, int yo)
{
    upload();
    if (tilewise) buildTilewise();
    last_B = input.B;
    ciphertext3D out(input.B, zo, xo, yo, out_form);
    if (streamed) { stream_form = forwardStreamed(input, out); return out; }
    size_t wb = crc_conv2d_forms_work_bytes(ctx(), input.B, zd, xd, yd, xs, ys, xf, yf, nf, input.form, w_form, out_form);
    if (!wb) throw invalid_argument(kind() + string(": unsupported geometry"));
    ensure(g_scratch, wb);
    chk(crc_conv2d_forms(ctx(), input.data(), (const uint64_t *)d_w->ptr, w_form, (const uint64_t *)d_b[out_form != CRC_COEFF]->ptr, input.B, zd, xd, yd, xs,
        ys, xf, yf, nf, input.form, out_form, out.data(), g_scratch->ptr, stream()), dense ? "crc_dense_forms" : "crc_conv2d_forms");
    if (out_form == CRC_NTTLC) out.form = CRC_NTTL;
    return out;
}
int MacLayer::forwardStreamed(const ciphertext3D &input, ciphertext3D &out)
{
    const size_t n = N(), k = K(), rowb = k * n * 8, ctb = ctBytes();
    const size_t T = taps(), P = (size_t)((xd - xf) / xs + 1) * ((yd - yf) / ys + 1);
    auto scatter = [&](int f0, int ft) {
        for (int b = 0; b < input.B; b++)
            chk(crc_memcpy_d2d(ctx(), (char *)out.buf->ptr + ((size_t)b * nf + f0) * P * ctb, (const char *)d_ytile->ptr + (size_t)b * ft * P * ctb,
                (size_t)ft * P * ctb, stream()), "crc_memcpy_d2d");
    };
    const bool ntt_in = input.form == CRC_NTT || input.form == CRC_NTTP || input.form == CRC_NTTL;
    if (ntt_in && plannedForm(input.B) == CRC_NTTL) {
        const int ft_max = min(64, nf), sub = min(8, ft_max);
        const size_t wt = (size_t)sub * T * rowb, wl = crc_limb_weights_bytes(ctx(), ft_max, zd, xf, yf), yt = (size_t)input.B * ft_max * P * ctb;
        ensure(d_wtile, wt);
        ensure(d_ytile, yt);
        ensure(g_wltile, wl);
        const void *xl = input.data();
        if (input.form != CRC_NTTL) {
            const size_t xb = crc_limb_tensor_bytes(ctx(), input.B, zd, xd, yd);
            ensure(g_xltile, xb);
            chk(crc_limb_pack_tensor(ctx(), input.data(), input.form, input.B, zd, xd, yd, g_xltile->ptr, stream()), "crc_limb_pack_tensor");
            xl = g_xltile->ptr;
        }
        const size_t wb = crc_conv2d_forms_work_bytes(ctx(), input.B, zd, xd, yd, xs, ys, xf, yf, ft_max, CRC_NTTL, CRC_NTTL, out_form);
        ensure(g_scratch, wb);
// ... 620 lines not shown
        fused->d_w = make_shared<DeviceBuffer>((size_t)conv.nf * conv.zd * xf2 * yf2 * rowb);
        fused->d_b[1] = make_shared<DeviceBuffer>((size_t)conv.nf * rowb);
        chk(crc_conv2d_fold_pool(ctx(), (const uint64_t *)conv.d_w->ptr, (const uint64_t *)conv.d_b[1]->ptr, div ? (const uint64_t *)div->ptr : nullptr,
                                 conv.nf, conv.zd, conv.xf, conv.yf, conv.xs, conv.ys, pxf, pyf, (uint64_t *)fused->d_w->ptr, (uint64_t *)fused->d_b[1]->ptr,
                                 stream()), "crc_conv2d_fold_pool");
        fused->d_b[0] = inttCopy(fused->d_b[1], conv.nf);
        fused->filters_already_ntt = true;
        return fused;
    };
    for (size_t i = 0; i + 1 < layers.size(); i++) {
        auto conv = dynamic_pointer_cast<ConvolutionalLayer>(layers[i]);
        auto pool = dynamic_pointer_cast<PoolingLayer>(layers[i + 1]);
        if (!conv || !pool || refreshBetween(i)) continue;
        conv->upload();
        if (conv->streamed) continue;
        if (pool->zd != conv->nf || pool->xd != conv->xo || pool->yd != conv->yo) continue;
        const int xf2 = (pool->xf - 1) * conv->xs + conv->xf, yf2 = (pool->yf - 1) * conv->ys + conv->yf;
        const int xs2 = conv->xs * pool->xs, ys2 = conv->ys * pool->ys;
        if (xf2 > conv->xd || yf2 > conv->yd) continue;
        const int xo2 = (conv->xd - xf2) / xs2 + 1, yo2 = (conv->yd - yf2) / ys2 + 1;
        if (xo2 != pool->xo || yo2 != pool->yo) continue;
        int fold = 0;
        chk(crc_plan_fold_pool(ctx(), conv->zd, conv->xd, conv->yd, conv->xs, conv->ys, conv->xf, conv->yf, conv->nf, pool->xs, pool->ys, pool->xf, pool->yf,
            &fold), "crc_plan_fold_pool");
        if (!fold) continue;
        auto up = i > 0 && !refreshBetween(i - 1) ? dynamic_pointer_cast<ConvolutionalLayer>(layers[i - 1]) : nullptr;
        if (up) { up->upload(); if (up->streamed || up->tilewise) up = nullptr; }
        int hoist = 0;
        chk(crc_plan_hoist_pool(ctx(), up ? up->zd : 0, up ? up->xd : 0, up ? up->yd : 0, up ? up->xs : 0, up ? up->ys : 0, up ? up->xf : 0, up ? up->yf : 0,
            up ? up->nf : 0, conv->zd, conv->xd, conv->yd, conv->xs, conv->ys, conv->xf, conv->yf, conv->nf, pool->xs, pool->ys, pool->xf, pool->yf,
            g_expected_batch, matrix_cores ? 1 : 0, &hoist), "crc_plan_hoist_pool");
        if (hoist) {
            auto sums = foldPool(*up, up->name, 1, 1, pool->xf, pool->yf, nullptr);
            vector<Plaintext> nob; plaintext4D nof;
            auto down = make_shared<ConvolutionalLayer>(conv->name + "+" + pool->name, sums->xo, sums->yo, conv->zd, pool->xs, pool->ys, conv->xf, conv->yf,
                conv->nf, conv->th_count, nof, nob);
            down->d_w = make_shared<DeviceBuffer>((size_t)conv->nf * conv->zd * conv->xf * conv->yf * rowb);
            down->d_b[1] = make_shared<DeviceBuffer>((size_t)conv->nf * rowb);
            chk(crc_conv2d_hoist_pool(ctx(), (const uint64_t *)conv->d_w->ptr, (const uint64_t *)conv->d_b[1]->ptr, pool->d_div ?
                (const uint64_t *)pool->d_div->ptr : nullptr, conv->nf, conv->zd, conv->xf, conv->yf, pool->xf, pool->yf, (uint64_t *)down->d_w->ptr,
                (uint64_t *)down->d_b[1]->ptr, stream()), "crc_conv2d_hoist_pool");
            down->d_b[0] = inttCopy(down->d_b[1], conv->nf);
            down->filters_already_ntt = true;
            layers[i - 1] = sums;
            layers[i] = down;
            eraseLayer(i + 1);
            continue;
        }
        layers[i] = foldPool(*conv, conv->name + "+" + pool->name, pool->xs, pool->ys, pool->xf, pool->yf, pool->d_div);
        eraseLayer(i + 1);
    }
    for (size_t i = 0; i + 1 < layers.size(); i++) {
        auto sq = dynamic_pointer_cast<SquareLayer>(layers[i]);
        auto pool = dynamic_pointer_cast<PoolingLayer>(layers[i + 1]);
        if (!sq || !pool || refreshBetween(i)) continue;
        if (!crc_square_pool_relin_supported(ctx(), 16, pool->xf, pool->yf)) continue;
        layers[i] = make_shared<SquarePoolLayer>(sq->name + "+" + pool->name, pool->xd, pool->yd, pool->zd, pool->xs, pool->ys, pool->xf, pool->yf,
            sq->th_count,
                                                 pool->d_div);
        eraseLayer(i + 1);
    }
    for (size_t i = 0; i + 1 < layers.size(); i++) {
        auto po = dynamic_pointer_cast<PolyLayer>(layers[i]);
        auto pool = dynamic_pointer_cast<PoolingLayer>(layers[i + 1]);
        if (!po || !pool || refreshBetween(i)) continue;
        if (!crc_poly2_pool_relin_supported(ctx(), 16, pool->xf, pool->yf)) continue;
        auto pp = make_shared<PolyPoolLayer>(po->name + "+" + pool->name, pool->xd, pool->yd, pool->zd, pool->xs, pool->ys, pool->xf, pool->yf, po->th_count,
                                             po->c2, po->c1, po->c0, pool->d_div);
        for (int j = 0; j < 3; j++) pp->slot_scale[j] = po->slot_scale[j];
        layers[i] = pp;
        eraseLayer(i + 1);
    }
    for (size_t i = 0; i + 1 < layers.size(); i++) {
        auto bn = dynamic_pointer_cast<BatchNormLayer>(layers[i]);
        if (!bn || refreshBetween(i)) continue;
        auto m = dynamic_pointer_cast<MacLayer>(layers[i + 1]);
        if (!m) continue;
        const int ch = bn->num_channels, T = (int)m->taps();
        if (m->dense ? T % ch != 0 : m->zd != ch) continue;
        const int per_ch = T / ch;
        m->upload();
        if (m->streamed) continue;
        bn->upload();
        if (m->tilewise) {
            if (m->tile_built) continue;
            m->fold_bn = bn;
            m->name = bn->name + "+" + m->name;
            eraseLayer(i);
            continue;
        }
        BnFold fold(*bn, T, per_ch, m->nf);
        vector<uint64_t> bias = m->hostBias();
        fold.apply((uint64_t *)m->d_w->ptr, m->nf, bias.data());
        m->setBias(bias);
        m->name = bn->name + "+" + m->name;
        eraseLayer(i);
    }
    chk(crc_stream_sync(ctx(), stream()), "crc_stream_sync");
    if (removed) fused_ = true;
    return removed;
}

namespace {
const struct { const char *name, *text; } kBuiltinModels[] = {
#include "builtin_models.inc"
};
[[noreturn]] void descError(int line, const string &what) { throw invalid_argument("line " + to_string(line) + ": " + what); }
float descFloat(int line, const string &tok, const char *what)
{
    char *end = nullptr;
// ... 358 lines not shown
```

crcnn_amd/host/crcnn_host.h:

```cpp
#pragma once
#include <cstdint>
#include <istream>
#include <memory>
#include <ostream>
#include <stdexcept>
#include <string>
#include <utility>
#include <vector>
#include "../../include/crcnn_hip.h"

class Plaintext {
public:
    int coeff_count_ = 0;
    std::vector<std::pair<int, uint64_t>> nz;
    int coeff_count() const { return coeff_count_; }
    bool is_zero() const { return nz.empty(); }
    void save(std::ostream &stream) const;
    void load(std::istream &stream);
    void dense(uint64_t *out, int n) const;
};
typedef std::vector<std::vector<std::vector<Plaintext>>> plaintext3D;
typedef std::vector<std::vector<Plaintext>> plaintext2D;
typedef std::vector<std::vector<std::vector<std::vector<Plaintext>>>> plaintext4D;
typedef std::vector<std::vector<std::vector<std::vector<float>>>> floatHypercube;
// ... 71 lines not shown

class Layer {
public:
    std::string name;
    int out_form = CRC_COEFF;
    Layer() {}
    Layer(std::string layer_name) : name(layer_name) {}
    virtual ~Layer() {}
    std::string getName() { return name; }
    virtual void printLayerStructure() = 0;
    virtual ciphertext3D forward(ciphertext3D input) = 0;
    virtual void savePlaintextParameters(std::ostream *outfile) = 0;
    virtual void loadPlaintextParameters(std::istream *infile) = 0;
    void computeBoundaries(int xd, int yd, int xs, int ys, int xf, int yf, int *xl, int *yl);
    virtual void deviceParameters(std::vector<std::shared_ptr<DeviceBuffer>> &out, bool allocate_only) { (void)out; (void)allocate_only; }
    virtual int placement() { return 0; }
    virtual void adoptPlacement(int p) { (void)p; }
    virtual size_t deviceBytes() const { return 0; }
    virtual std::string kernelName() const { return ""; }
};

class BatchNormLayer;
struct BnFold;
class MacLayer : public Layer {
public:
    friend class Network;
    const int zd, xd, yd, xs, ys, xf, yf, nf;
    void deviceParameters(std::vector<std::shared_ptr<DeviceBuffer>> &out, bool allocate_only) override;
    int placement() override;
    void adoptPlacement(int p) override { forced_placement = p; }
    void restoreCanonical();
    size_t deviceBytes() const override;
    std::string kernelName() const override;
protected:
    MacLayer(std::string name, bool dense, int zd, int xd, int yd, int xs, int ys, int xf, int yf, int nf)
        : Layer(name), zd(zd), xd(xd), yd(yd), xs(xs), ys(ys), xf(xf), yf(yf), nf(nf), dense(dense), slot_weights(slotEncoding()) {}
    ciphertext3D run(const ciphertext3D &input, int zo, int xo, int yo);
private:
    virtual bool &alreadyNtt() = 0;
    virtual bool hasPlaintexts() const = 0;
    virtual void plaintexts(int f0, int fn, std::vector<const Plaintext *> &w, std::vector<const Plaintext *> *b) const = 0;
    const bool dense;
    const char *kind() const { return dense ? "FullyConnectedLayer" : "ConvolutionalLayer"; }
    size_t taps() const { return (size_t)zd * xf * yf; }
    std::shared_ptr<DeviceBuffer> d_w, d_b[2];
    bool streamed = false;
    int stream_form = CRC_NTT;
    std::shared_ptr<DeviceBuffer> d_plain, d_wtile, d_ytile;
    int w_form = CRC_NTT;
    bool slot_weights;
    std::shared_ptr<DeviceBuffer> d_w_canon;
    bool tilewise = false, tile_built = false;
    std::shared_ptr<BatchNormLayer> fold_bn;
    int last_B = 0;
    int forced_placement = -1;
    bool forcedTilewise() const { return dense && forced_placement == 2; }
    int plannedForm(int B) const;
    bool limbFits() const;
    void upload();
    void buildTilewise();
    void packWeights(bool unpack);
    bool limbWeights(int B);
    bool streamsOnMatrixCores(int B);
    int forwardStreamed(const ciphertext3D &input, ciphertext3D &out);
    std::vector<uint64_t> hostBias();
    void setBias(const std::vector<uint64_t> &ntt_rows);
};

class ConvolutionalLayer : public MacLayer {
public:
    int th_count;
    int xo, yo, zo;
    plaintext4D filters;
    std::vector<Plaintext> biases;
    bool filters_already_ntt = false;
    ConvolutionalLayer(std::string name, int xd, int yd, int zd, int xs, int ys, int xf, int yf, int nf, int th_count, plaintext4D &filters,
        std::vector<Plaintext> &biases);
// ... 276 lines not shown
```

crcnn_amd/netrun.py:

```python
import math
import os

import numpy as np

from . import binding
from .binding import COEFF, NTT

TOPOLOGIES = {
    "PlainModelTiny": [
        ("conv", "pool1_features.conv1", dict(xd=28, yd=28, zd=1, xs=1, ys=1, xf=5, yf=5, nf=32)),
        ("avgpool", "pool1", dict(xd=24, yd=24, zd=32, xs=2, ys=2, xf=2, yf=2)),
        ("conv", "pool2_features.conv2", dict(xd=12, yd=12, zd=32, xs=1, ys=1, xf=5, yf=5, nf=64)),
        ("avgpool", "pool2", dict(xd=8, yd=8, zd=64, xs=2, ys=2, xf=2, yf=2)),
        ("fc", "classifier.fc3", dict(in_dim=1024, out_dim=512)),
        ("fc", "classifier.fc4", dict(in_dim=512, out_dim=10)),
    ],
    "ApproxPlainModel": [
        ("conv", "pool1_features.conv1", dict(xd=28, yd=28, zd=1, xs=2, ys=2, xf=5, yf=5, nf=20)),
        ("avgpool", "pool1", dict(xd=12, yd=12, zd=20, xs=1, ys=1, xf=2, yf=2)),
        ("bn", "pool1_features.norm1", dict(ch=20)),
        ("conv", "pool2_features.conv2", dict(xd=11, yd=11, zd=20, xs=2, ys=2, xf=3, yf=3, nf=50)),
        ("square", "act1", dict()),
        ("avgpool", "pool2", dict(xd=5, yd=5, zd=50, xs=1, ys=1, xf=2, yf=2)),
        ("bn", "pool2_features.norm2", dict(ch=50)),
# ... 302 lines not shown
            elif kind == "pad":
                p["form"] = form
            elif kind == "square":
                p["in_form"] = form
                p["out_form"] = COEFF if (last or not resident) else NTT
                form = p["out_form"]
            elif kind == "poly":
                p["in_form"] = form
                p["out_form"] = COEFF if (last or not resident) else NTT
                form = p["out_form"]
                if eng.device >= 0:
                    p["rows"] = eng.poly2_rows(a["c2"], a["c1"], a["c0"])
                    self._keep_rows(p["rows"])
            elif kind == "poly3":
                p["in_form"] = form
                p["out_form"] = COEFF if (last or not resident) else NTT
                form = p["out_form"]
                if eng.device >= 0:
                    p["rows"] = eng.poly3_rows(a["c3"], a["c2"], a["c1"], a["c0"])
                    self._keep_rows(p["rows"])
            nshape = out_shape(kind, a, shape)
            self.plan.append((kind, name, a, p, shape, nshape))
            shape = nshape
        self.out_shape = shape
        self.out_form = form
        self._packed = False
        if self.fuse_pool:
            self.fuse()

    @staticmethod
    def _geom(kind, a):
        return (a["zd"], a["xd"], a["yd"], a["xs"], a["ys"], a["xf"], a["yf"], a["nf"]) if kind == "conv" else (a["in_dim"], 1, 1, 1, 1, 1, 1, a["out_dim"])

    def planned_form(self, kind, a, B=0):
        if kind not in ("conv", "fc"):
            return NTT
        wf = self.E.plan_mac(*self._geom(kind, a), B, matrix_cores=self.limb)
        if wf == binding.NTTL1 and os.environ.get("CRC_MFMA_CONV1", "1") == "0":
            wf = binding.NTTP
        return wf

    def limb_eligible(self, kind, a):
        return self.planned_form(kind, a, 0) == binding.NTTL

    def conv1_eligible(self, kind, a):
        return self.planned_form(kind, a, 0) == binding.NTTL1

    def _needs_tilewise(self, kind, a, count):
        E = self.E
        nf, zd, xf, yf = (a["nf"], a["zd"], a["xf"], a["yf"]) if kind == "conv" else (a["out_dim"], a["in_dim"], 1, 1)
        canon, limb = count * E_k_n_8(E), E.limb_weights_bytes(nf, zd, xf, yf)
        free = E.mem_info()[0]
        return canon + limb + self.limb_reserve > free and limb + self.limb_reserve + (8 << 30) <= free

    def _build_tilewise(self):
        E = self.E
        if not self.materialize:
            return
        rowb = E.k * E.n * 8
        for (kind, name, a, p, ishape, oshape) in self.plan:
            tw = p.get("tilewise")
            want = "folded" if p.get("bn_fold") else "plain"
            if not tw or tw["built"] == want:
                continue
            assert tw["built"] is False or want == "folded", "a batch-norm fold cannot be taken back"
            nf, zd, xf, yf = (a["nf"], a["zd"], a["xf"], a["yf"]) if kind == "conv" else (a["out_dim"], a["in_dim"], 1, 1)
# ... 15 lines not shown
                qv = np.array(E.q, dtype=np.uint64).reshape(1, E.k, 1)
            for f0 in range(0, nf, ft):
                fn = min(ft, nf - f0)
                vals = np.ascontiguousarray(wv[f0:f0 + fn]).reshape(-1)
                for o in range(0, vals.size, chunk):
                    cnt = E.encode_to_device(vals[o:o + chunk], stage, cstage)
                    E.plain_to_ntt(stage, cnt, E.p(wt) + o * rowb)
                    E.sync()
                if bn:
                    for f in range(fn):
                        E.L.crc_multiply_plain_ntt(E.c, E.p(wt) + f * T * rowb, E.p(bn["invstd"]), T, bn["per_ch"], 1, E.stream)
                    E.dense(fake, wt, None, 1, T, fn, NTT, NTT, outc, wk)
                    E.sync()
                    corr = E.download(E.p(outc), (fn, 2, E.k, E.n))[:, 0]
                    bias[f0:f0 + fn] = (bias[f0:f0 + fn] + (qv - corr)) % qv
                E.limb_pack_weights_tile(wt, nf, f0, fn, zd, xf, yf, p["w"])
                E.sync()
            if bn:
                bias = np.ascontiguousarray(bias)
                E.L.crc_memcpy_h2d(E.c, E.p(p["b"]), bias.ctypes.data, bias.nbytes, E.stream)
                E.sync()
                for b_ in (fake, outc, wk):
                    self._free(b_)
            self._free(wt); self._free(stage); self._free(cstage)
            tw["built"] = want

    def _limb_operands(self, B=None, B_tail=None, split=None):
        E = self.E
        if self._limbed or not self.limb:
            return
        assert not self._packed
        self._build_tilewise()
        for idx, (kind, name, a, p, ishape, oshape) in enumerate(self.plan):
            if self.conv1_eligible(kind, a) and not p.get("streamed"):
                nbytes = E.limb_conv1_weights_bytes_for(a["nf"], a["xf"], a["yf"])
                wl = self.alloc(nbytes)
                E.limb_conv1_pack_weights(p["w"], a["nf"], a["xf"], a["yf"], wl)
                E.sync()
                self.weight_bytes += nbytes - a["nf"] * a["xf"] * a["yf"] * E.k * E.n * 8
                self._free(p["w"])
                p["w"], p["w_form"] = wl, binding.NTTL1
                continue
            if not self.limb_eligible(kind, a) or p.get("streamed") or p.get("tilewise"):
                continue
            Bl = B if (B_tail is None or split is None or idx < split) else B_tail
            if Bl is not None and self.planned_form(kind, a, Bl) != binding.NTTL:
                p["limb_skipped"] = "fewer than 32 rows per launch"
                continue
            nf, zd, xf, yf = (a["nf"], a["zd"], a["xf"], a["yf"]) if kind == "conv" else (a["out_dim"], a["in_dim"], 1, 1)
            nbytes = E.limb_weights_bytes(nf, zd, xf, yf)
            if E.mem_info()[0] < nbytes + self.limb_reserve:
                p["limb_skipped"] = f"limb copy of {nbytes >> 30} GiB + {self.limb_reserve >> 30} GiB reserve > {E.mem_info()[0] >> 30} GiB free"
                continue
            wl = self.alloc(nbytes)
            E.limb_pack_weights(p["w"], nf, zd, xf, yf, wl)
            E.sync()
            self.weight_bytes += nbytes - nf * zd * xf * yf * E.k * E.n * 8
            self._free(p["w"])
            p["w"], p["w_form"] = wl, binding.NTTL
        for idx, (kind, name, a, p, ishape, oshape) in enumerate(self.plan):
            nxt = self.plan[idx + 1] if idx + 1 < len(self.plan) else None
            if p.get("w_form") == binding.NTTL and nxt and nxt[0] == "fc" and nxt[3].get("w_form") == binding.NTTL and p["out_form"] == NTT and nxt[3]["in_form"] == NTT:
                p["out_form"] = nxt[3]["in_form"] = binding.NTTL
            if p.get("w_form") == binding.NTTL1 and nxt and nxt[0] == "conv" and nxt[3].get("w_form") == binding.NTTL and p["out_form"] == NTT and nxt[3]["in_form"] == NTT:
                p["out_form"], nxt[3]["in_form"] = binding.NTTLC, binding.NTTL
        self._limbed = True

    def _free(self, buf):
        self.param_bufs = [(b_, n_) for (b_, n_) in self.param_bufs if b_ is not buf]
        if getattr(self, "release", None):
            self.release(buf)
        elif hasattr(buf, "free"):
            buf.free()

    def _pack_operands(self, unpack=False):
        E = self.E
        if unpack:
            assert not self._limbed, "fuse() must run before the weights are converted to limb form"
        if max(int(q).bit_length() for q in E.q) > 55 or self._packed == (not unpack):
            return
        for idx, (kind, name, a, p, ishape, oshape) in enumerate(self.plan):
            if kind in ("pool", "avgpool"):
                nxt = self.plan[idx + 1] if idx + 1 < len(self.plan) else None
                if nxt and nxt[0] in ("conv", "fc"):
                    if not unpack and p["form"] == NTT and nxt[3]["in_form"] == NTT:
                        p["form"] = nxt[3]["in_form"] = binding.NTTP
                    elif unpack and p["form"] == binding.NTTP:
                        p["form"] = nxt[3]["in_form"] = NTT
                continue
            if kind not in ("conv", "fc"):
                continue
            if p.get("w_form") not in (binding.NTTL, binding.NTTL1) and not p.get("streamed"):
                rows = (a["nf"] * a["zd"] * a["xf"] * a["yf"] if kind == "conv" else a["in_dim"] * a["out_dim"]) * E.k
                E.pack28(p["w"], rows, unpack=unpack)
                p["w_form"] = NTT if unpack else binding.NTTP
            nxt = self.plan[idx + 1] if idx + 1 < len(self.plan) else None
            if nxt and nxt[0] in ("conv", "fc"):
                if not unpack and p["out_form"] == NTT and nxt[3]["in_form"] == NTT:
                    p["out_form"] = nxt[3]["in_form"] = binding.NTTP
                elif unpack and p["out_form"] == binding.NTTP:
                    p["out_form"] = nxt[3]["in_form"] = NTT
        E.sync()
        self._packed = not unpack

    def fuse(self):
        E = self.E
        if self.materialize:
            self._pack_operands(unpack=True)
        plan, i = [], 0
        while i < len(self.plan):
            kind, name, a, p, ishape, oshape = self.plan[i]
            nxt = self.plan[i + 1] if i + 1 < len(self.plan) else None
            if kind == "conv" and not p.get("streamed") and not p.get("tilewise") and nxt and nxt[0] in ("pool", "avgpool") and p["out_form"] == NTT and nxt[3]["form"] == NTT:
                pa = nxt[2]
                xf2, yf2 = (pa["xf"] - 1) * a["xs"] + a["xf"], (pa["yf"] - 1) * a["ys"] + a["yf"]
                xs2, ys2 = a["xs"] * pa["xs"], a["ys"] * pa["ys"]
                xo2, yo2 = (a["xd"] - xf2) // xs2 + 1, (a["yd"] - yf2) // ys2 + 1
                macs_sep = layer_macs("conv", a)
                macs_fused = a["nf"] * xo2 * yo2 * a["zd"] * xf2 * yf2
                same_shape = (a["nf"], xo2, yo2) == tuple(nxt[5])
                if same_shape and E.plan_fold_pool(a["zd"], a["xd"], a["yd"], a["xs"], a["ys"], a["xf"], a["yf"], a["nf"], pa["xs"], pa["ys"], pa["xf"], pa["yf"]):
                    up = plan[-1] if plan and plan[-1][0] == "conv" and not plan[-1][3].get("streamed") and not plan[-1][3].get("tilewise") and plan[-1][3]["out_form"] == NTT else None
                    if E.plan_hoist_pool(self._geom("conv", up[2]) if up else None, self._geom("conv", a), (pa["xs"], pa["ys"], pa["xf"], pa["yf"]), 0, matrix_cores=self.limb):
                        plan[-1] = self._fold_sum_pool(up, pa["xf"], pa["yf"])
                        sshape = plan[-1][5]
                        cnt = a["nf"] * a["zd"] * a["xf"] * a["yf"]
                        w2 = self.alloc(cnt * E.k * E.n * 8); b2 = self.alloc(a["nf"] * E.k * E.n * 8)
                        if self.materialize:
                            E.conv2d_hoist_pool(p["w"], p["b"], nxt[3]["div"], a["nf"], a["zd"], a["xf"], a["yf"], pa["xf"], pa["yf"], w2, b2)
                            E.sync()
                        self.param_bufs = [(b_, n_) for (b_, n_) in self.param_bufs if b_ is not p["w"] and b_ is not p["b"]]
                        self.param_bufs += [(w2, cnt * E.k * E.n * 8), (b2, a["nf"] * E.k * E.n * 8)]
                        a2 = dict(a, xd=sshape[1], yd=sshape[2], xs=pa["xs"], ys=pa["ys"])
                        p2 = dict(p, w=w2, b=b2, fused=(name, nxt[1]), macs_separate=macs_sep, macs=layer_macs("conv", a2))
                        p["w"] = p["b"] = None
                        plan.append(("conv", name + "+" + nxt[1], a2, p2, sshape, nxt[5]))
                        i += 2
                        continue
                    cnt = a["nf"] * a["zd"] * xf2 * yf2
                    w2 = self.alloc(cnt * E.k * E.n * 8); b2 = self.alloc(a["nf"] * E.k * E.n * 8)
                    if self.materialize:
                        E.conv2d_fold_pool(p["w"], p["b"], nxt[3]["div"], a["nf"], a["zd"], a["xf"], a["yf"], a["xs"], a["ys"], pa["xf"], pa["yf"], w2, b2)
                        E.sync()
                    self.param_bufs = [(b_, n_) for (b_, n_) in self.param_bufs if b_ is not p["w"] and b_ is not p["b"]]
                    self.param_bufs += [(w2, cnt * E.k * E.n * 8), (b2, a["nf"] * E.k * E.n * 8)]
                    self.weight_bytes += (cnt - a["nf"] * a["zd"] * a["xf"] * a["yf"]) * E.k * E.n * 8
                    a2 = dict(a, xs=xs2, ys=ys2, xf=xf2, yf=yf2)
                    p2 = dict(p, w=w2, b=b2, fused=(name, nxt[1]), macs_separate=macs_sep, macs=macs_fused)
                    p["w"] = p["b"] = None
                    plan.append(("conv", name + "+" + nxt[1], a2, p2, ishape, nxt[5]))
                    i += 2
                    continue
            plan.append(self.plan[i]); i += 1
        self.plan = plan
        self._pair_square_pool()
        self._fold_batchnorm()

    def _fold_sum_pool(self, entry, pxf, pyf):
        E = self.E
        kind, name, a, p, ishape, oshape = entry
        xf2, yf2 = (pxf - 1) * a["xs"] + a["xf"], (pyf - 1) * a["ys"] + a["yf"]
        cnt = a["nf"] * a["zd"] * xf2 * yf2
        w2 = self.alloc(cnt * E.k * E.n * 8); b2 = self.alloc(a["nf"] * E.k * E.n * 8)
        if self.materialize:
            E.conv2d_fold_pool(p["w"], p["b"], None, a["nf"], a["zd"], a["xf"], a["yf"], a["xs"], a["ys"], pxf, pyf, w2, b2)
            E.sync()
        self.param_bufs = [(b_, n_) for (b_, n_) in self.param_bufs if b_ is not p["w"] and b_ is not p["b"]]
        self.param_bufs += [(w2, cnt * E.k * E.n * 8), (b2, a["nf"] * E.k * E.n * 8)]
        self.weight_bytes += (cnt - a["nf"] * a["zd"] * a["xf"] * a["yf"]) * E.k * E.n * 8
        a2 = dict(a, xf=xf2, yf=yf2)
        p2 = dict(p, w=w2, b=b2, macs=layer_macs("conv", a2))
        return (kind, name, a2, p2, ishape, (oshape[0], oshape[1] - pxf + 1, oshape[2] - pyf + 1))

    def _keep_rows(self, rows):
        rowb = self.E.k * self.E.n * 8
        for r in rows:
            if r is not None:
                self.weight_bytes += rowb
                self.param_bufs.append((r, rowb))

    def _pair_square_pool(self):
        E = self.E
        plan, i = [], 0
        while i < len(self.plan):
            kind, name, a, p, ishape, oshape = self.plan[i]
            nxt = self.plan[i + 1] if i + 1 < len(self.plan) else None
            if (kind == "square" and nxt and nxt[0] in ("pool", "avgpool") and p["out_form"] == NTT and nxt[3]["form"] == NTT
                    and E.square_pool_relin_supported(nxt[2]["xf"], nxt[2]["yf"], self.dbc)):
                plan.append(("squarepool", name + "+" + nxt[1], dict(nxt[2]), dict(in_form=p["in_form"], out_form=NTT, div=nxt[3]["div"]), ishape, nxt[5]))
                i += 2
                continue
            if (kind == "poly" and nxt and nxt[0] in ("pool", "avgpool") and p["out_form"] == NTT and nxt[3]["form"] == NTT
                    and E.poly2_pool_relin_supported(nxt[2]["xf"], nxt[2]["yf"], self.dbc)):
                rows = (None, None, None)
                if E.device >= 0:
                    old = [r for r in p.get("rows", ()) if r is not None]
                    self.param_bufs = [(b_, n_) for (b_, n_) in self.param_bufs if not any(b_ is r for r in old)]
                    self.weight_bytes -= len(old) * E.k * E.n * 8
                    rows = E.poly2_rows(a["c2"], a["c1"], a["c0"], window=nxt[2]["xf"] * nxt[2]["yf"], d_div=nxt[3]["div"])
                    self._keep_rows(rows)
                plan.append(("polypool", name + "+" + nxt[1], dict(nxt[2]), dict(in_form=p["in_form"], out_form=NTT, rows=rows), ishape, nxt[5]))
                i += 2
                continue
            plan.append(self.plan[i]); i += 1
        self.plan = plan

    def _fold_batchnorm(self):
        E = self.E
        plan, i = [], 0
        rowb = E.k * E.n * 8
        while i < len(self.plan):
            kind, name, a, p, ishape, oshape = self.plan[i]
            nxt = self.plan[i + 1] if i + 1 < len(self.plan) else None
            if kind == "bn" and nxt and nxt[0] in ("conv", "fc") and p["form"] == NTT and nxt[3]["out_form"] == NTT and "fused" not in nxt[3] and not nxt[3].get("streamed"):
                nk, nname, na, np_, nish, nosh = nxt
                ch = ishape[0]
                if nk == "conv":
                    F, per_ch, T = na["nf"], na["xf"] * na["yf"], na["zd"] * na["xf"] * na["yf"]
                else:
                    F, per_ch, T = na["out_dim"], ishape[1] * ishape[2], na["in_dim"]
                assert T == ch * per_ch
                if np_.get("tilewise"):
                    np_["bn_fold"] = dict(mean=p["mean"], invstd=p["invstd"], ch=ch, per_ch=per_ch)
                elif self.materialize:
                    for f in range(F):
                        E.L.crc_multiply_plain_ntt(E.c, E.p(np_["w"]) + f * T * rowb, E.p(p["invstd"]), T, per_ch, 1, E.stream)
                    fake = self.alloc(T * 2 * rowb); outc = self.alloc(F * 2 * rowb)
                    E.L.crc_memset(E.c, E.p(fake), 0, T * 2 * rowb, E.stream)
                    for z in range(ch):
                        for t in range(per_ch):
                            E.L.crc_memcpy_d2d(E.c, E.p(fake) + (z * per_ch + t) * 2 * rowb, E.p(p["mean"]) + z * rowb, rowb, E.stream)
                    wk = self.alloc(max(E.dense_work_bytes(1, T, F, NTT), 256))
                    E.dense(fake, np_["w"], None, 1, T, F, NTT, NTT, outc, wk)
                    E.sync()
                    corr = E.download(E.p(outc), (F, 2, E.k, E.n))[:, 0]
                    bias = E.download(E.p(np_["b"]), (F, E.k, E.n))
                    qv = np.array(E.q, dtype=np.uint64).reshape(1, E.k, 1)
                    newb = np.ascontiguousarray((bias + (qv - corr)) % qv)
                    E.L.crc_memcpy_h2d(E.c, E.p(np_["b"]), newb.ctypes.data, newb.nbytes, E.stream)
                    E.sync()
                    self._keep.append(newb)
                self.param_bufs = [(b_, n_) for (b_, n_) in self.param_bufs if b_ is not p["mean"] and b_ is not p["invstd"]]
                self.weight_bytes -= 2 * ch * rowb
                p2 = dict(np_, folded_bn=name)
                plan.append((nk, name + "+" + nname, na, p2, ishape, nosh))
                i += 2
                continue
# ... 50 lines not shown
        self.weight_bytes += len(pl) * E.k * E.n * 8
        self.param_bufs.append((out, len(pl) * E.k * E.n * 8))
        if not self.materialize:
            return out
        d_p = self.alloc(pl.nbytes)
        E.L.crc_memcpy_h2d(E.c, E.p(d_p), pl.ctypes.data, pl.nbytes, E.stream)
        E.plain_to_delta(d_p, len(pl), form, out)
        E.sync()
        return out

    def ct_bytes(self):
        return 2 * self.E.k * self.E.n * 8

    def activation_cts(self):
        return [int(np.prod(s)) for (_, _, _, _, s, _) in self.plan] + [int(np.prod(self.out_shape))]

    def scratch_bytes(self, B):
        E = self.E
        acts = self.activation_cts()
        big = sorted(acts, reverse=True)
        need_act = (big[0] + big[1]) * B * self.ct_bytes()
        work = 0
        B0 = B
        for li, (kind, name, a, p, ishape, oshape) in enumerate(self.plan):
            B = B0 * getattr(self, "G", 1) if li >= getattr(self, "split", len(self.plan)) else B0
            if p.get("streamed"):
                g = self._stream_geometry(kind, a, B)
                if g["limb"]:
                    fin = binding.NTTL if p["in_form"] in (NTT, binding.NTTP, binding.NTTL) else p["in_form"]
                    work = max(work, E.conv2d_forms_work_bytes(B, g["zd"], g["xd"], g["yd"], g["xs"], g["ys"], g["xf"], g["yf"], g["ft"], fin, binding.NTTL, p["out_form"]))
                else:
                    work = max(work, E.conv2d_forms_work_bytes(B, g["zd"], g["xd"], g["yd"], g["xs"], g["ys"], g["xf"], g["yf"], g["ft"], p["in_form"], NTT, p["out_form"]))
                continue
            if kind == "conv":
                work = max(work, E.conv2d_forms_work_bytes(B, a["zd"], a["xd"], a["yd"], a["xs"], a["ys"], a["xf"], a["yf"], a["nf"], p["in_form"], p.get("w_form", NTT), p["out_form"]))
            elif kind == "fc":
                work = max(work, E.conv2d_forms_work_bytes(B, a["in_dim"], 1, 1, 1, 1, 1, 1, a["out_dim"], p["in_form"], p.get("w_form", NTT), p["out_form"]))
            elif kind == "square":
                work = max(work, E.square_relin_work_bytes(B * int(np.prod(ishape)), self.dbc))
            elif kind == "squarepool":
                work = max(work, E.square_pool_relin_work_bytes(B, a["zd"], a["xd"], a["yd"], a["xs"], a["ys"], a["xf"], a["yf"], self.dbc))
            elif kind == "poly":
                work = max(work, E.poly2_relin_work_bytes(B * int(np.prod(ishape)), self.dbc))
            elif kind == "poly3":
                work = max(work, E.poly3_relin_work_bytes(B * int(np.prod(ishape)), self.dbc))
            elif kind == "polypool":
                work = max(work, E.poly2_pool_relin_work_bytes(B, a["zd"], a["xd"], a["yd"], a["xs"], a["ys"], a["xf"], a["yf"], self.dbc))
        return need_act, work

    def _stream_geometry(self, kind, a, B=None):
        g = dict(zd=a["zd"], xd=a["xd"], yd=a["yd"], xs=a["xs"], ys=a["ys"], xf=a["xf"], yf=a["yf"], nf=a["nf"]) if kind == "conv" else \
            dict(zd=a["in_dim"], xd=1, yd=1, xs=1, ys=1, xf=1, yf=1, nf=a["out_dim"])
        T = g["zd"] * g["xf"] * g["yf"]
        g["T"] = T
        g["P"] = ((g["xd"] - g["xf"]) // g["xs"] + 1) * ((g["yd"] - g["yf"]) // g["ys"] + 1)
        g["limb"] = bool(self.limb and B is not None and self.planned_form(kind, a, B) == binding.NTTL)
        if g["limb"]:
            g["ft"] = min(64, g["nf"]); g["sub"] = min(8, g["ft"])
            return g
        if not hasattr(self, "_stream_tile_bytes"):
            self._stream_tile_bytes = max(2 << 30, min(16 << 30, self.E.mem_info()[0] // 8))
        ft = self._stream_tile_bytes // (T * self.E.k * self.E.n * 8)
        g["ft"] = max(1, min(g["nf"], ft // 8 * 8 if ft >= 8 else ft))
        return g

    def _forward_streamed(self, kind, a, p, cur, B, out):
        E = self.E
# ... 104 lines not shown

    def forward(self, d_x, B, timer=None):
        assert self.G == 1, "prepared for two-level chunking: use forward_group"
        return self._run(0, len(self.plan), d_x, B, self.buf, timer)

    def forward_group(self, d_xs, B, timer=None):
        E = self.E
        if self.G == 1:
            assert len(d_xs) == 1
            return self._run(0, len(self.plan), d_xs[0], B, self.buf, timer)
        assert 1 <= len(d_xs) <= self.G
        Bt = len(d_xs) * B
        for c, d_x in enumerate(d_xs):
            if self.tail_limb:
                cur = self._run(0, self.split, d_x, B, self.buf, timer)
                E.limb_pack_tensor_at(cur, self.tail_limb["form"], B, self.tail_limb["ch"], 1, 1, self.tail_in, Bt, c * B)
            else:
                self._run(0, self.split, d_x, B, self.buf, timer, last_out=E.p(self.tail_in) + c * B * self.tail_in_img)
        return self._run(self.split, len(self.plan), self.tail_in, Bt, self.tail_buf, timer)

    def _run(self, lo, hi, d_x, B, bufs, timer=None, last_out=None):
        E = self.E
        cur = d_x
        for i in range(lo, hi):
            kind, name, a, p, ishape, oshape = self.plan[i]
            out = bufs[self.slots[i]]
            if last_out is not None and i == hi - 1 and kind != "bn":
                out = last_out
            if timer:
                timer(i, name, kind, 0)
            if p.get("streamed"):
                self._forward_streamed(kind, a, p, cur, B, out)
                cur = out
            elif kind == "conv":
                E.conv2d(cur, p["w"], p["b"], B, a["zd"], a["xd"], a["yd"], a["xs"], a["ys"], a["xf"], a["yf"], a["nf"], p["in_form"], p["out_form"], out, self.work,
                         w_form=p.get("w_form", NTT))
                cur = out
            elif kind == "fc":
                E.dense(cur, p["w"], p["b"], B, a["in_dim"], a["out_dim"], p["in_form"], p["out_form"], out, self.work, w_form=p.get("w_form", NTT))
                cur = out
            elif kind in ("pool", "avgpool"):
                E.pool(cur, B, a["zd"], a["xd"], a["yd"], a["xs"], a["ys"], a["xf"], a["yf"], p["div"], p["form"], out)
                cur = out
            elif kind == "pad":
                E.pad(cur, B, a["zd"], a["xd"], a["yd"], a["px"], a["px"], a["py"], a["py"], p["form"], out)
                cur = out
            elif kind == "bn":
                if E.p(cur) != E.p(out):
                    E.L.crc_memcpy_d2d(E.c, E.p(out), E.p(cur), B * int(np.prod(ishape)) * self.ct_bytes(), E.stream)
                    cur = out
                E.batchnorm(cur, B, ishape[0], ishape[1], ishape[2], p["mean"], p["invstd"], p["form"])
            elif kind == "square":
                E.square_relin(cur, B * int(np.prod(ishape)), self.d_evk, out, self.work, self.dbc, p["in_form"], p["out_form"])
                cur = out
            elif kind == "squarepool":
                E.square_pool_relin(cur, B, a["zd"], a["xd"], a["yd"], a["xs"], a["ys"], a["xf"], a["yf"], self.d_evk, out, self.work, self.dbc, p["in_form"], p["out_form"],
                                    d_div=p["div"])
                cur = out
            elif kind == "poly":
                E.poly2_relin(cur, B * int(np.prod(ishape)), self.d_evk, *p["rows"], out, self.work, self.dbc, p["in_form"], p["out_form"])
                cur = out
            elif kind == "poly3":
                E.poly3_relin(cur, B * int(np.prod(ishape)), self.d_evk, *p["rows"], out, self.work, self.dbc, p["in_form"], p["out_form"])
                cur = out
            elif kind == "polypool":
                E.poly2_pool_relin(cur, B, a["zd"], a["xd"], a["yd"], a["xs"], a["ys"], a["xf"], a["yf"], self.d_evk, *p["rows"], out, self.work, self.dbc,
# ... 8 lines not shown
```

include/crcnn_hip.h:

```cpp
#ifndef CRCNN_HIP_H
#define CRCNN_HIP_H
#include <stddef.h>
#include <stdint.h>

#ifdef __cplusplus
extern "C" {
#endif

typedef struct crc_ctx crc_ctx;

typedef enum {
    CRC_OK = 0,
    CRC_ERR_INVALID_ARGUMENT = -1,
    CRC_ERR_PARAMETERS = -2,
    CRC_ERR_HIP = -3,
    CRC_ERR_UNSUPPORTED = -4,
    CRC_ERR_IO = -5,
    CRC_ERR_NOT_FOUND = -6,
    CRC_ERR_COMM = -7
} crc_status;

enum { CRC_COEFF = 0, CRC_NTT = 1,
       CRC_NTTP = 2,
       CRC_NTTL = 3,
// ... 55 lines not shown
int crc_ntt_inv_bsk(crc_ctx *ctx, uint64_t *d_rows, size_t count, void *stream);

int crc_add(crc_ctx *ctx, uint64_t *d_acc, const uint64_t *d_b, size_t count, int size, void *stream);
int crc_add_plain(crc_ctx *ctx, uint64_t *d_ct, const uint64_t *d_delta, size_t count, size_t group, int sign, void *stream);
int crc_multiply_plain_ntt(crc_ctx *ctx, uint64_t *d_ct, const uint64_t *d_w_ntt, size_t count, size_t group, int size, void *stream);
int crc_multiply_plain(crc_ctx *ctx, uint64_t *d_ct, const uint64_t *d_w_ntt, size_t count, size_t group, void *stream);

size_t crc_conv2d_work_bytes(const crc_ctx *ctx, int B, int zd, int xd, int yd, int xs, int ys, int xf, int yf, int nf, int in_form);
int crc_conv2d(crc_ctx *ctx, const uint64_t *d_x, const uint64_t *d_w_ntt, const uint64_t *d_bias_delta,
               int B, int zd, int xd, int yd, int xs, int ys, int xf, int yf, int nf,
               int in_form, int out_form, uint64_t *d_y, void *d_work, void *stream);
int crc_conv2d_fold_pool(crc_ctx *ctx, const uint64_t *d_w_ntt, const uint64_t *d_bias_delta_ntt, const uint64_t *d_div_ntt, int nf, int zd, int xf, int yf,
                         int cxs, int cys, int pxf, int pyf, uint64_t *d_w_out, uint64_t *d_bias_out, void *stream);
int crc_conv2d_hoist_pool(crc_ctx *ctx, const uint64_t *d_w_ntt, const uint64_t *d_bias_delta_ntt, const uint64_t *d_div_ntt, int nf, int zd, int xf, int yf,
                          int pxf, int pyf, uint64_t *d_w_out, uint64_t *d_bias_out, void *stream);
int crc_conv2d_forms(crc_ctx *ctx, const uint64_t *d_x, const uint64_t *d_w_ntt, int w_form, const uint64_t *d_bias_delta,
                     int B, int zd, int xd, int yd, int xs, int ys, int xf, int yf, int nf,
                     int in_form, int out_form, uint64_t *d_y, void *d_work, void *stream);
int crc_dense_forms(crc_ctx *ctx, const uint64_t *d_x, const uint64_t *d_w_ntt, int w_form, const uint64_t *d_bias_delta,
                    int B, int in_dim, int out_dim, int in_form, int out_form, uint64_t *d_y, void *d_work, void *stream);
int    crc_limb_supported(const crc_ctx *ctx, int zd, int xf, int yf);
size_t crc_limb_tensor_bytes(const crc_ctx *ctx, int B, int zd, int xd, int yd);
size_t crc_limb_weights_bytes(const crc_ctx *ctx, int nf, int zd, int xf, int yf);
int    crc_limb_pack_weights(crc_ctx *ctx, const uint64_t *d_w_ntt, int nf, int zd, int xf, int yf, void *d_wl, void *stream);
int    crc_limb_pack_weights_tile(crc_ctx *ctx, const uint64_t *d_w_tile_ntt, int nf, int f0, int ft, int zd, int xf, int yf, void *d_wl, void *stream);
int    crc_plan_mac(const crc_ctx *ctx, int zd, int xd, int yd, int xs, int ys, int xf, int yf, int nf, int B, int matrix_cores, int *w_form);
size_t crc_scalar_weights_bytes(const crc_ctx *ctx, int nf, int zd, int xf, int yf);
int    crc_scalar_supported(const crc_ctx *ctx, int B, int zd, int xd, int yd, int xs, int ys, int xf, int yf, int nf);
int    crc_scalar_pack_weights(crc_ctx *ctx, const uint64_t *d_w, int w_stride, int nf, int zd, int xf, int yf, void *d_ws, int *constant, void *stream);
int    crc_plan_mac_scalar(const crc_ctx *ctx, int zd, int xd, int yd, int xs, int ys, int xf, int yf, int nf, int B, int *w_form);
int    crc_plan_fold_pool(const crc_ctx *ctx, int zd, int xd, int yd, int xs, int ys, int xf, int yf, int nf, int pxs, int pys, int pxf, int pyf, int *fold);
int    crc_plan_hoist_pool(const crc_ctx *ctx, int uzd, int uxd, int uyd, int uxs, int uys, int uxf, int uyf, int unf, int zd, int xd, int yd, int xs, int ys,
                           int xf, int yf, int nf, int pxs, int pys, int pxf, int pyf, int B, int matrix_cores, int *hoist);
int    crc_limb_pack_tensor(crc_ctx *ctx, const uint64_t *d_x, int in_form, int B, int zd, int xd, int yd, void *d_xl, void *stream);
int    crc_limb_pack_tensor_at(crc_ctx *ctx, const uint64_t *d_x, int in_form, int B, int zd, int xd, int yd, void *d_xl, int Btot, int b0, void *stream);
int    crc_limb_conv1_supported(const crc_ctx *ctx, int zd, int xd, int yd, int xs, int ys, int xf, int yf, int nf);
size_t crc_limb_conv1_weights_bytes(const crc_ctx *ctx);
size_t crc_limb_conv1_weights_bytes_for(const crc_ctx *ctx, int nf, int xf, int yf);
int    crc_limb_conv1_form(const crc_ctx *ctx, int zd, int xd, int yd, int xs, int ys, int xf, int yf, int nf);
int    crc_limb_conv1_pack_weights(crc_ctx *ctx, const uint64_t *d_w_ntt, int nf, int xf, int yf, void *d_wl, void *stream);
size_t crc_conv2d_forms_work_bytes(const crc_ctx *ctx, int B, int zd, int xd, int yd, int xs, int ys, int xf, int yf, int nf, int in_form, int w_form,
int out_form);
int crc_pack28(crc_ctx *ctx, uint64_t *d_rows, size_t rows, int unpack, void *stream);
size_t crc_dense_work_bytes(const crc_ctx *ctx, int B, int in_dim, int out_dim, int in_form);
int crc_dense(crc_ctx *ctx, const uint64_t *d_x, const uint64_t *d_w_ntt, const uint64_t *d_bias_delta,
              int B, int in_dim, int out_dim, int in_form, int out_form, uint64_t *d_y, void *d_work, void *stream);
int crc_pool(crc_ctx *ctx, const uint64_t *d_x, int B, int zd, int xd, int yd, int xs, int ys, int xf, int yf,
             const uint64_t *d_div_ntt , int form, uint64_t *d_y, void *stream);
int crc_batchnorm(crc_ctx *ctx, uint64_t *d_x, int B, int zd, int xd, int yd, const uint64_t *d_mean_delta,
                  const uint64_t *d_invstd_ntt, int form, void *stream);
int crc_pad(crc_ctx *ctx, const uint64_t *d_x, int B, int zd, int xd, int yd, int px0, int px1, int py0, int py1, int form, uint64_t *d_y, void *stream);
size_t crc_square_relin_work_bytes(const crc_ctx *ctx, size_t count, int dbc);
int crc_square_relin(crc_ctx *ctx, const uint64_t *d_x, size_t count, const uint64_t *d_evk, int dbc,
                     uint64_t *d_y, void *d_work, void *stream);
int crc_square_relin_forms(crc_ctx *ctx, const uint64_t *d_x, int in_form, size_t count, const uint64_t *d_evk, int dbc,
                           uint64_t *d_y, int out_form, void *d_work, void *stream);
int    crc_square_pool_relin_supported(const crc_ctx *ctx, int dbc, int xf, int yf);
size_t crc_square_pool_relin_work_bytes(const crc_ctx *ctx, int B, int zd, int xd, int yd, int xs, int ys, int xf, int yf, int dbc);
int    crc_square_pool_relin_forms(crc_ctx *ctx, const uint64_t *d_x, int in_form, int B, int zd, int xd, int yd, int xs, int ys, int xf, int yf,
                                   const uint64_t *d_evk, int dbc, const uint64_t *d_div_ntt , uint64_t *d_y, int out_form, void *d_work,
                                   void *stream);
size_t crc_poly2_relin_work_bytes(const crc_ctx *ctx, size_t count, int dbc);
int    crc_poly2_relin_forms(crc_ctx *ctx, const uint64_t *d_x, int in_form, size_t count, const uint64_t *d_evk, int dbc, const uint64_t *d_p2_ntt,
                             const uint64_t *d_p1_ntt, const uint64_t *d_p0_ntt, uint64_t *d_y, int out_form, void *d_work, void *stream);
int    crc_poly2_pool_relin_supported(const crc_ctx *ctx, int dbc, int xf, int yf);
size_t crc_poly2_pool_relin_work_bytes(const crc_ctx *ctx, int B, int zd, int xd, int yd, int xs, int ys, int xf, int yf, int dbc);
// ... 148 lines not shown
```

Baseline: 799.9.

## Box-sum conv1 inputs instead of enlarging filters when folding sum-pool

When a sum-pool is folded into the first convolution, the new path keeps the original small filter and instead box-sums shifted input ciphertexts during the limb row-packing step, avoiding an enlarged filter. A planner compares the estimated MAC cost of the enlarged filter against the boxed cost plus the extra input reads, and picks the cheaper one. It is enabled by default through a tune flag. The packing kernel gains a templated box branch with additional global reads and modular reductions, and the cost constant for the plain conv1 path is also adjusted slightly.

```diff
diff --git a/crcnn_amd/binding.py b/crcnn_amd/binding.py
--- a/crcnn_amd/binding.py
+++ b/crcnn_amd/binding.py
@@ -134,6 +134,10 @@
     L.crc_plan_hoist_pool.argtypes = [VP] + [CI] * 22 + [ctypes.POINTER(CI)]
     L.crc_limb_pack_tensor.argtypes = [VP, VP, CI, CI, CI, CI, CI, VP, VP]
     L.crc_limb_conv1_supported.argtypes = [VP] + [CI] * 8
+    L.crc_limb_conv1_box_supported.argtypes = [VP] + [CI] * 10
+    L.crc_conv2d_box_forms_work_bytes.restype = SZ; L.crc_conv2d_box_forms_work_bytes.argtypes = [VP] + [CI] * 14
+    L.crc_conv2d_box_forms.argtypes = [VP, VP, VP, CI, VP] + [CI] * 11 + [CI, CI, VP, VP, VP]
+    L.crc_plan_conv1_box.argtypes = [VP] + [CI] * 12 + [ctypes.POINTER(CI)]
     L.crc_limb_conv1_weights_bytes.restype = SZ; L.crc_limb_conv1_weights_bytes.argtypes = [VP]
     L.crc_limb_conv1_pack_weights.argtypes = [VP, VP, CI, CI, CI, VP, VP]
     L.crc_limb_conv1_weights_bytes_for.restype = SZ; L.crc_limb_conv1_weights_bytes_for.argtypes = [VP, CI, CI, CI]
@@ -615,6 +619,22 @@
              "crc_plan_hoist_pool")
         return bool(h.value)
 
+    def limb_conv1_box_supported(self, zd, xd, yd, xs, ys, xf, yf, nf, bxf, byf):
+        return bool(self.L.crc_limb_conv1_box_supported(self.c, zd, xd, yd, xs, ys, xf, yf, nf, bxf, byf))
+
+    def conv2d_box_forms_work_bytes(self, B, zd, xd, yd, xs, ys, xf, yf, nf, bxf, byf, in_form, w_form, out_form):
+        return self.L.crc_conv2d_box_forms_work_bytes(self.c, B, zd, xd, yd, xs, ys, xf, yf, nf, bxf, byf, in_form, w_form, out_form)
+
+    def conv2d_box(self, d_x, d_w, d_bias, B, zd, xd, yd, xs, ys, xf, yf, nf, bxf, byf, in_form, out_form, d_y, d_work, w_form=NTTL1):
+        _chk(self.L.crc_conv2d_box_forms(self.c, self.p(d_x), self.p(d_w), w_form, self.p(d_bias), B, zd, xd, yd, xs, ys, xf, yf, nf, bxf, byf, in_form, out_form,
+                                         self.p(d_y), self.p(d_work), self.stream), "crc_conv2d_box_forms")
+
+    def plan_conv1_box(self, zd, xd, yd, xs, ys, xf, yf, nf, bxf, byf, B=0, matrix_cores=True):
+        b = CI(0)
+        _chk(self.L.crc_plan_conv1_box(self.c, zd, xd, yd, xs, ys, xf, yf, nf, bxf, byf, int(B or 0), 1 if matrix_cores else 0, ctypes.byref(b)),
+             "crc_plan_conv1_box")
+        return bool(b.value)
+
     def scalar_weights_bytes(self, nf, zd, xf=1, yf=1):
         return self.L.crc_scalar_weights_bytes(self.c, nf, zd, xf, yf)
 
diff --git a/crcnn_amd/csrc/abi.hip b/crcnn_amd/csrc/abi.hip
--- a/crcnn_amd/csrc/abi.hip
+++ b/crcnn_amd/csrc/abi.hip
@@ -157,23 +157,24 @@
     return (int)(fit < 1 ? 1 : fit > (size_t)B ? (size_t)B : fit);
 }
 struct Limb1Work { signed char *Xr; u64 *Ys, *buf; int Bs, out_form; };
-static Limb1Work limb1_layout(const crc_ctx *c, int B, int xd, int yd, int xf, int yf, int nf, int P, int in_form, int out_form, WorkArena &a)
+static Limb1Work limb1_layout(const crc_ctx *c, int B, int xd, int yd, int xdi, int ydi, int xf, int yf, int nf, int P, int in_form, int out_form, WorkArena &a)
 {
     Limb1Work L{};
     L.out_form = out_form == CRC_NTTLC && P == 1 ? CRC_NTTL : out_form;
-    L.Bs = conv1_sub_batch(c, B, xd, yd, xf, yf, nf, P, L.out_form);
-    L.Xr = a.take<signed char>(k_limb_conv1_image_bytes(c, L.Bs, xd, yd, xf, yf, nf));
+    L.Bs = conv1_sub_batch(c, B, xdi, ydi, xf, yf, nf, P, L.out_form);
+    L.Xr = a.take<signed char>(k_limb_conv1_image_bytes(c, L.Bs, xdi, ydi, xf, yf, nf));
     if (L.out_form != CRC_NTTLC) L.Ys = a.take<u64>(k_limb_result_words(c, L.Bs, nf, P));
     if (in_form == CRC_COEFF) L.buf = a.take<u64>((size_t)L.Bs * xd * yd * crc_ct_words(c, 2));
     return L;
 }
 static int conv2d_limb1(crc_ctx *c, const uint64_t *d_x, const void *d_wl, const uint64_t *d_bias, int B, int xd, int yd, int xs, int ys, int xf, int yf,
     int nf,
-                        int in_form, int out_form, uint64_t *d_y, void *d_work, hipStream_t st)
-{
-    const int xo = (xd - xf) / xs + 1, yo = (yd - yf) / ys + 1, P = xo * yo, in_cts = xd * yd;
+                        int in_form, int out_form, uint64_t *d_y, void *d_work, hipStream_t st, int bxf = 1, int byf = 1)
+{
+    const int xdi = xd - (bxf - 1) * xs, ydi = yd - (byf - 1) * ys;
+    const int xo = (xdi - xf) / xs + 1, yo = (ydi - yf) / ys + 1, P = xo * yo, in_cts = xd * yd;
     WorkArena a(d_work);
-    const Limb1Work L = limb1_layout(c, B, xd, yd, xf, yf, nf, P, in_form, out_form, a);
+    const Limb1Work L = limb1_layout(c, B, xd, yd, xdi, ydi, xf, yf, nf, P, in_form, out_form, a);
     out_form = L.out_form;
     const size_t ctw = crc_ct_words(c, 2);
     for (int b0 = 0; b0 < B; b0 += L.Bs) {
@@ -182,7 +183,7 @@
         if (in_form == CRC_COEFF) { RUN(k_ntt_ct(c, false, xn, L.buf, (size_t)Bn * in_cts, 2, false, st, nullptr, 0, 0, 0, 0)); xn = L.buf; packed = false; }
         RUN(k_limb_conv1(c, xn, packed, L.Xr, (const signed char *)d_wl, L.Ys, out_form == CRC_NTTLC ? (signed char *)d_y : nullptr, B, b0,
             out_form != CRC_COEFF ? d_bias : nullptr,
-                         Bn, xd, yd, xs, ys, xf, yf, nf, st));
+                         Bn, xd, yd, xs, ys, xf, yf, nf, st, bxf, byf));
         if (out_form == CRC_NTTLC) continue;
         if (out_form == CRC_NTTL) return k_limb_result_to_limb(c, L.Ys, (signed char *)d_y, B, nf * P, st);
         RUN(k_limb_result_to_rows(c, L.Ys, d_y + (size_t)b0 * nf * P * ctw, (size_t)Bn * nf * P * 2, out_form == CRC_NTTP, st));
@@ -205,7 +206,7 @@
     if (!c || !conv_shape_ok(xd, yd, xs, ys, xf, yf)) return 0;
     const int P = ((xd - xf) / xs + 1) * ((yd - yf) / ys + 1);
     WorkArena a;
-    if (w_form == CRC_NTTL1) limb1_layout(c, B, xd, yd, xf, yf, nf, P, in_form, out_form, a);
+    if (w_form == CRC_NTTL1) limb1_layout(c, B, xd, yd, xd, yd, xf, yf, nf, P, in_form, out_form, a);
     else if (w_form == CRC_NTTL || w_form == CRC_NTTLS) limb_layout(c, B, zd, xd, yd, nf, P, in_form, a);
     else conv_layout(c, B, zd, xd, yd, xf, yf, P, in_form, a);
     return a.bytes();
@@ -286,6 +287,35 @@
         RUN(k_ntt_ct(c, true, d_y, d_y, (size_t)B * nf * P, 2, false, st, d_bias, 1, (size_t)P, nf));
     return CRC_OK;
 }
+extern "C" int crc_limb_conv1_box_supported(const crc_ctx *c, int zd, int xd, int yd, int xs, int ys, int xf, int yf, int nf, int bxf, int byf)
+{
+    if (!c || nf < 1 || bxf < 1 || byf < 1 || xs < 1 || ys < 1) return 0;
+    const int xdi = xd - (bxf - 1) * xs, ydi = yd - (byf - 1) * ys;
+    if (!conv_shape_ok(xd, yd, xs, ys, xf, yf) || !conv_shape_ok(xdi, ydi, xs, ys, xf, yf)) return 0;
+    return k_limb_conv1_box_shape(c, zd, xd, yd, xs, ys, xf, yf, nf, bxf, byf) ? 1 : 0;
+}
+extern "C" size_t crc_conv2d_box_forms_work_bytes(const crc_ctx *c, int B, int zd, int xd, int yd, int xs, int ys, int xf, int yf, int nf, int bxf, int byf,
+    int in_form, int w_form, int out_form)
+{
+    if (c && bxf == 1 && byf == 1) return crc_conv2d_forms_work_bytes(c, B, zd, xd, yd, xs, ys, xf, yf, nf, in_form, w_form, out_form);
+    if (w_form != CRC_NTTL1 || !crc_limb_conv1_box_supported(c, zd, xd, yd, xs, ys, xf, yf, nf, bxf, byf)) return 0;
+    const int xdi = xd - (bxf - 1) * xs, ydi = yd - (byf - 1) * ys, P = ((xdi - xf) / xs + 1) * ((ydi - yf) / ys + 1);
+    WorkArena a;
+    limb1_layout(c, B, xd, yd, xdi, ydi, xf, yf, nf, P, in_form, out_form, a);
+    return a.bytes();
+}
+extern "C" int crc_conv2d_box_forms(crc_ctx *c, const uint64_t *d_x, const uint64_t *d_w, int w_form, const uint64_t *d_bias, int B, int zd, int xd, int yd,
+                                    int xs, int ys, int xf, int yf, int nf, int bxf, int byf, int in_form, int out_form, uint64_t *d_y, void *d_work,
+                                    void *stream)
+{
+    if (bxf == 1 && byf == 1) return crc_conv2d_forms(c, d_x, d_w, w_form, d_bias, B, zd, xd, yd, xs, ys, xf, yf, nf, in_form, out_form, d_y, d_work, stream);
+    CHECK_CTX(c);
+    if (!d_x || !d_w || !d_y || !d_work || B < 0 || nf < 1 || bxf < 1 || byf < 1 || !nform_ok(in_form) || !(lform_ok(out_form) || out_form == CRC_NTTLC) ||
+        !conv_shape_ok(xd, yd, xs, ys, xf, yf)) return CRC_ERR_INVALID_ARGUMENT;
+    if (w_form != CRC_NTTL1 || !crc_limb_conv1_box_supported(c, zd, xd, yd, xs, ys, xf, yf, nf, bxf, byf)) return CRC_ERR_UNSUPPORTED;
+    if (B == 0) return CRC_OK;
+    return conv2d_limb1(c, d_x, d_w, d_bias, B, xd, yd, xs, ys, xf, yf, nf, in_form, out_form, d_y, d_work, S(stream), bxf, byf);
+}
 extern "C" int crc_conv2d(crc_ctx *c, const uint64_t *d_x, const uint64_t *d_w, const uint64_t *d_bias, int B, int zd, int xd, int yd,
                           int xs, int ys, int xf, int yf, int nf, int in_form, int out_form, uint64_t *d_y, void *d_work, void *stream)
 {
@@ -438,7 +468,7 @@
     int wf = CRC_NTT;
     if (crc_plan_mac(c, zd, xd, yd, xs, ys, xf, yf, nf, B, matrix_cores, &wf) != CRC_OK) return -1;
     const long long P = (long long)((xd - xf) / xs + 1) * ((yd - yf) / ys + 1);
-    if (wf == CRC_NTTL1) return 32 * ((2 * P + 15) / 16 * 8) * ((k_limb_conv1_form(c, xf, yf, nf) == 2 ? 40 : 64) + 24) * 25 / 16;
+    if (wf == CRC_NTTL1) return 32 * ((2 * P + 15) / 16 * 8) * ((k_limb_conv1_form(c, xf, yf, nf) == 2 ? 40 : 64) + 24) * 8 / 5;
     if (wf == CRC_NTTL) return (long long)(nf + 31) / 32 * 32 * P * ((long long)k_limb_steps(zd, xf, yf) * 32 + 24);
     return (long long)(nf + 7) / 8 * 8 * P * ((long long)zd * xf * yf + 24);
 }
@@ -470,6 +500,25 @@
     return CRC_OK;
 }
 
+#define PLAN_BOX_READ 21
+extern "C" int crc_plan_conv1_box(const crc_ctx *c, int zd, int xd, int yd, int xs, int ys, int xf, int yf, int nf, int bxf, int byf, int B, int matrix_cores,
+                                  int *box)
+{
+    if (!c || !box || zd < 1 || nf < 1 || bxf < 1 || byf < 1 || !conv_shape_ok(xd, yd, xs, ys, xf, yf)) return CRC_ERR_INVALID_ARGUMENT;
+    *box = 0;
+    if (!c->tune.conv1_box || !matrix_cores || bxf * byf == 1) return CRC_OK;
+    if (!crc_limb_conv1_box_supported(c, zd, xd, yd, xs, ys, xf, yf, nf, bxf, byf)) return CRC_OK;
+    const int xf2 = (bxf - 1) * xs + xf, yf2 = (byf - 1) * ys + yf, xdi = xd - (bxf - 1) * xs, ydi = yd - (byf - 1) * ys;
+    if (!conv_shape_ok(xd, yd, xs, ys, xf2, yf2)) return CRC_OK;
+    int wf = CRC_NTT;
+    if (crc_plan_mac(c, zd, xdi, ydi, xs, ys, xf, yf, nf, B, matrix_cores, &wf) != CRC_OK || wf != CRC_NTTL1) return CRC_OK;
+    const long long enlarged = plan_mac_cost(c, zd, xd, yd, xs, ys, xf2, yf2, nf, B, matrix_cores);
+    const long long boxed = plan_mac_cost(c, zd, xdi, ydi, xs, ys, xf, yf, nf, B, matrix_cores) +
+                            (long long)xdi * ydi * 2 * (bxf * byf - 1) * PLAN_BOX_READ;
+    *box = enlarged >= 0 && boxed < enlarged ? 1 : 0;
+    return CRC_OK;
+}
+
 static size_t square_chunk(const crc_ctx *c)
 {
     if (c->tune.sq_chunk > 0) return (size_t)c->tune.sq_chunk;
diff --git a/crcnn_amd/csrc/ctx.cpp b/crcnn_amd/csrc/ctx.cpp
--- a/crcnn_amd/csrc/ctx.cpp
+++ b/crcnn_amd/csrc/ctx.cpp
@@ -164,6 +164,7 @@
     t.conv1_narrow = (int)geti("CRC_CONV1_NARROW", 1);
     { const int v = (int)geti("CRC_CONV1_FORM", 0); t.conv1_form = v == 1 || v == 2 ? v : 0; }
     t.hoist_pool = geti("CRC_HOIST_POOL", 1) ? 1 : 0;
+    t.conv1_box = geti("CRC_CONV1_BOX", 1) ? 1 : 0;
     { const long long v = geti("CRC_CONV1_PASS_BYTES", 0); t.conv1_pass_bytes = v > 0 ? v : 0; }
     { const int v = (int)geti("CRC_LIMB_PACK_GROUP", 1); t.limb_pack_group = v > 0 ? v : 1; }
     t.mac2_cfg = (int)geti("CRC_MAC2_CFG", 0);
@@ -196,6 +197,7 @@
     else if (s == "conv1_narrow") t.conv1_narrow = (int)value;
     else if (s == "conv1_form") t.conv1_form = value == 1 || value == 2 ? (int)value : 0;
     else if (s == "hoist_pool") t.hoist_pool = value ? 1 : 0;
+    else if (s == "conv1_box") t.conv1_box = value ? 1 : 0;
     else if (s == "conv1_pass_bytes") t.conv1_pass_bytes = value > 0 ? value : 0;
     else if (s == "limb_pack_group") t.limb_pack_group = value > 0 ? (int)value : 1;
     else if (s == "mac2_cfg") t.mac2_cfg = (int)value;
diff --git a/crcnn_amd/csrc/ctx.h b/crcnn_amd/csrc/ctx.h
--- a/crcnn_amd/csrc/ctx.h
+++ b/crcnn_amd/csrc/ctx.h
@@ -86,6 +86,7 @@
     int mfma_ring = 0;
     int conv1_waves = 0;
     int conv1_narrow = 1;
+    int conv1_box = 1;
     int hoist_pool = 1;
     int conv1_form = 0;
     long long conv1_pass_bytes = 0;
diff --git a/crcnn_amd/csrc/kernels.h b/crcnn_amd/csrc/kernels.h
--- a/crcnn_amd/csrc/kernels.h
+++ b/crcnn_amd/csrc/kernels.h
@@ -105,4 +105,5 @@
 size_t k_limb_conv1_image_bytes(const crc_ctx *c, int B, int xd, int yd, int xf, int yf, int nf);
 int k_limb_conv1_pack_weights(crc_ctx *c, const u64 *w, signed char *wl, int nf, int xf, int yf, hipStream_t st);
 int k_limb_conv1(crc_ctx *c, const u64 *x, bool packed, signed char *xr, const signed char *wl, u64 *ys, signed char *xl_out, int Bout, int b0, const u64 *bias_ntt, int B, int xd, int yd,
-                 int xs, int ys_, int xf, int yf, int nf, hipStream_t st);
+                 int xs, int ys_, int xf, int yf, int nf, hipStream_t st, int bxf = 1, int byf = 1);
+bool   k_limb_conv1_box_shape(const crc_ctx *c, int zd, int xd, int yd, int xs, int ys_, int xf, int yf, int nf, int bxf, int byf);
diff --git a/crcnn_amd/csrc/kernels_mfma1.hip b/crcnn_amd/csrc/kernels_mfma1.hip
--- a/crcnn_amd/csrc/kernels_mfma1.hip
+++ b/crcnn_amd/csrc/kernels_mfma1.hip
@@ -353,36 +353,62 @@
         *reinterpret_cast<uint4 *>(dst) = *reinterpret_cast<const uint4 *>(st + (size_t)run * (RG * 32) + part * 16);
     }
 }
+template <bool BOX>
 __global__ void __launch_bounds__(256) limb_pack_rows1_kernel_px(const u64 *x, i8 *xr, const ModParams *mods, int n, int k, int B, int xd, int yd, int packed,
-                                                                 unsigned img_stride, unsigned poly_bytes, unsigned rs)
+                                                                 unsigned img_stride, unsigned poly_bytes, unsigned rs, int xdo, int ydo, int bxf, int byf, int xs,
+                                                                 int ys)
 {
     extern __shared__ __attribute__((aligned(16))) i8 stp[];
     const unsigned sstride = RG * rs + 16;
     const int sblocks = n / RSL;
     const int sb = blockIdx.x % (sblocks * k), i = sb / sblocks, s0 = (sb % sblocks) * RSL;
-    const int rgs = (xd + RG - 1) / RG;
+    const int rgs = (xdo + RG - 1) / RG;
     size_t r = blockIdx.x / (sblocks * k);
     const int rg = (int)(r % rgs); r /= rgs; const int c = (int)(r % 2); const int b = (int)(r / 2);
     const u64 q = mods[i].q;
     const int lane = threadIdx.x & (RSL - 1), qrow = (threadIdx.x >> 5) & (RG - 1), h = threadIdx.x >> 7, row = rg * RG + qrow;
-    if (row < xd) {
+    if (row < xdo) {
+        const size_t cs = (size_t)2 * k * n;
         const u64 *src = x + ((((size_t)b * xd * yd + (size_t)row * yd + h * 16) * 2 + c) * k + i) * (size_t)n + s0 + lane;
         u64 *sp = reinterpret_cast<u64 *>(stp + (size_t)lane * sstride + qrow * rs) + h * 16;
-#pragma unroll
-        for (int colx = 0; colx < 16; colx++) {
-            const int col = h * 16 + colx;
-            if ((unsigned)col * 8 >= rs) continue;
-            u64 dg = 0;
-            if (col < yd) {
-                u64 v = src[(size_t)colx * 2 * k * n];
-                if (packed) v = (v & 0xffffffffULL) | ((v >> 32) << 28);
-                dg = balanced_digit_bytes(v, q);
-            }
-            sp[colx] = dg;
+        if constexpr (!BOX) {
+#pragma unroll
+            for (int colx = 0; colx < 16; colx++) {
+                const int col = h * 16 + colx;
+                if ((unsigned)col * 8 >= rs) continue;
+                u64 dg = 0;
+                if (col < yd) {
+                    u64 v = src[(size_t)colx * cs];
+                    if (packed) v = (v & 0xffffffffULL) | ((v >> 32) << 28);
+                    dg = balanced_digit_bytes(v, q);
+                }
+                sp[colx] = dg;
+            }
+        } else {
+            u64 sum[16];
+#pragma unroll
+            for (int colx = 0; colx < 16; colx++) sum[colx] = 0;
+            for (int a = 0; a < bxf; a++)
+                for (int bb = 0; bb < byf; bb++) {
+                    const u64 *tp = src + ((size_t)a * xs * yd + (size_t)bb * ys) * cs;
+#pragma unroll
+                    for (int colx = 0; colx < 16; colx++)
+                        if (h * 16 + colx < ydo) {
+                            u64 v = tp[(size_t)colx * cs];
+                            if (packed) v = (v & 0xffffffffULL) | ((v >> 32) << 28);
+                            sum[colx] += v;
+                        }
+                }
+#pragma unroll
+            for (int colx = 0; colx < 16; colx++) {
+                const int col = h * 16 + colx;
+                if ((unsigned)col * 8 >= rs) continue;
+                sp[colx] = col < ydo ? balanced_digit_bytes(sum_reduce16(sum[colx], q), q) : 0;
+            }
         }
     }
     __syncthreads();
-    const int per_run = RG * rs / 16, valid = min(RG, xd - rg * RG) * (int)rs / 16;
+    const int per_run = RG * rs / 16, valid = min(RG, xdo - rg * RG) * (int)rs / 16;
     for (int o = threadIdx.x; o < RSL * per_run; o += 256) {
         const int sl = o / per_run, part = o - sl * per_run;
         if (part >= valid) continue;
@@ -448,6 +474,13 @@
     if (xo * yo > 1024) return false;
     return conv1_fits(k_limb_conv1_form(c, xf, yf, nf) == 2 ? conv1_px_img_stride(xd, yd) : conv1_img_stride(xd), xd, yd, xs, ys_, xf, yf);
 }
+bool k_limb_conv1_box_shape(const crc_ctx *c, int zd, int xd, int yd, int xs, int ys_, int xf, int yf, int nf, int bxf, int byf)
+{
+    if (bxf < 1 || byf < 1 || bxf * byf > 9) return false;
+    const int xdo = xd - (bxf - 1) * xs, ydo = yd - (byf - 1) * ys_;
+    if (xdo < xf || ydo < yf || !k_limb_conv1_shape(c, zd, xdo, ydo, xs, ys_, xf, yf, nf)) return false;
+    return bxf * byf == 1 || k_limb_conv1_form(c, xf, yf, nf) == 2;
+}
 static size_t conv1_form_weights_bytes(const crc_ctx *c, int form) { return (size_t)c->n * c->k * NPL * 32 * 64 * (form == 2 ? NJ : 1); }
 size_t k_limb_conv1_weights_bytes(const crc_ctx *c) { return conv1_form_weights_bytes(c, 2); }
 size_t k_limb_conv1_weights_bytes_for(const crc_ctx *c, int nf, int xf, int yf) { return conv1_form_weights_bytes(c, k_limb_conv1_form(c, xf, yf, nf)); }
@@ -472,12 +505,13 @@
     HIPCHK(hipGetLastError());
     return CRC_OK;
 }
-int k_limb_conv1(crc_ctx *c, const u64 *x, bool packed, i8 *xr, const i8 *wl, u64 *ys, i8 *xl_out, int Bout, int b0, const u64 *bias_ntt, int B, int xd,
-    int yd, int xs, int ys_,
-                 int xf, int yf, int nf, hipStream_t st)
+int k_limb_conv1(crc_ctx *c, const u64 *x, bool packed, i8 *xr, const i8 *wl, u64 *ys, i8 *xl_out, int Bout, int b0, const u64 *bias_ntt, int B, int xd_in,
+    int yd_in, int xs, int ys_,
+                 int xf, int yf, int nf, hipStream_t st, int bxf, int byf)
 {
     if (B == 0) return CRC_OK;
-    if (!k_limb_conv1_shape(c, 1, xd, yd, xs, ys_, xf, yf, nf)) return CRC_ERR_UNSUPPORTED;
+    if (!k_limb_conv1_box_shape(c, 1, xd_in, yd_in, xs, ys_, xf, yf, nf, bxf, byf)) return CRC_ERR_UNSUPPORTED;
+    const int xd = xd_in - (bxf - 1) * xs, yd = yd_in - (byf - 1) * ys_;
     const int xo = (xd - xf) / xs + 1, yo = (yd - yf) / ys_ + 1;
     const int form = k_limb_conv1_form(c, xf, yf, nf);
     Conv1Args a{};
@@ -493,8 +527,12 @@
         a.px_rs = conv1_px_rs(yd); a.poly_bytes = conv1_px_poly_bytes(xd, yd); a.img_stride = conv1_px_img_stride(xd, yd);
         a.px_taps = xf * yf; a.px_yf = yf;
         a.px_pair = yf % 2 == 0 && ys_ % 2 == 0 ? 1 : 0;
-        hipLaunchKernelGGL(limb_pack_rows1_kernel_px, dim3((unsigned)pack_blocks), dim3(256), RSL * (RG * a.px_rs + 16), st, x, xr, c->d_mods, c->n, c->k, B, xd,
-            yd, packed ? 1 : 0, a.img_stride, a.poly_bytes, a.px_rs);
+        if (bxf * byf > 1)
+            hipLaunchKernelGGL(limb_pack_rows1_kernel_px<true>, dim3((unsigned)pack_blocks), dim3(256), RSL * (RG * a.px_rs + 16), st, x, xr, c->d_mods, c->n, c->k,
+                B, xd_in, yd_in, packed ? 1 : 0, a.img_stride, a.poly_bytes, a.px_rs, xd, yd, bxf, byf, xs, ys_);
+        else
+            hipLaunchKernelGGL(limb_pack_rows1_kernel_px<false>, dim3((unsigned)pack_blocks), dim3(256), RSL * (RG * a.px_rs + 16), st, x, xr, c->d_mods, c->n, c->k,
+                B, xd_in, yd_in, packed ? 1 : 0, a.img_stride, a.poly_bytes, a.px_rs, xd, yd, 1, 1, xs, ys_);
         HIPCHK(hipGetLastError());
         const size_t lds = 2 * (size_t)a.img_stride + (xl_out ? a.out_img_bytes : 0);
         { const int rc = crc_ctx_ensure_lds(c, (const void *)mfma_conv1_kernel_px, lds); if (rc) return rc; }
diff --git a/crcnn_amd/csrc/limbred.h b/crcnn_amd/csrc/limbred.h
--- a/crcnn_amd/csrc/limbred.h
+++ b/crcnn_amd/csrc/limbred.h
@@ -153,6 +153,15 @@
     return ((u64)cv + 0x0080808080808080ULL) ^ 0x0080808080808080ULL;
 }
 
+CRC_HD u64 sum_reduce16(u64 s, u64 q)
+{
+    s -= s >= (q << 3) ? q << 3 : 0;
+    s -= s >= (q << 2) ? q << 2 : 0;
+    s -= s >= (q << 1) ? q << 1 : 0;
+    s -= s >= q ? q : 0;
+    return s;
+}
+
 inline u64 inverse_mod_2_64(u64 q) { u64 inv = q; for (int it = 0; it < 6; it++) inv *= 2 - q * inv; return inv; }
 
 inline void bias_to_multiple(u64 q, long long (&B)[13])
diff --git a/crcnn_amd/host/crcnn_host.cpp b/crcnn_amd/host/crcnn_host.cpp
--- a/crcnn_amd/host/crcnn_host.cpp
+++ b/crcnn_amd/host/crcnn_host.cpp
@@ -814,9 +814,21 @@
 int MacLayer::plannedForm(int B) const
 {
     int wf = CRC_NTT;
-    if (slot_weights && g_matrix_cores) chk(crc_plan_mac_scalar(ctx(), zd, xd, yd, xs, ys, xf, yf, nf, B, &wf), "crc_plan_mac_scalar");
-    else chk(crc_plan_mac(ctx(), zd, xd, yd, xs, ys, xf, yf, nf, B, g_matrix_cores ? 1 : 0, &wf), "crc_plan_mac");
+    const int xdi = xd - (bxf - 1) * xs, ydi = yd - (byf - 1) * ys;
+    if (slot_weights && g_matrix_cores) chk(crc_plan_mac_scalar(ctx(), zd, xdi, ydi, xs, ys, wxf(), wyf(), nf, B, &wf), "crc_plan_mac_scalar");
+    else chk(crc_plan_mac(ctx(), zd, xdi, ydi, xs, ys, wxf(), wyf(), nf, B, g_matrix_cores ? 1 : 0, &wf), "crc_plan_mac");
     return wf;
+}
+void MacLayer::unbox()
+{
+    if (!boxed()) return;
+    packWeights(true);
+    const size_t rowb = (size_t)K() * N() * 8;
+    auto w2 = make_shared<DeviceBuffer>((size_t)nf * zd * xf * yf * rowb), b2 = make_shared<DeviceBuffer>((size_t)nf * rowb);
+    chk(crc_conv2d_fold_pool(ctx(), (const uint64_t *)d_w->ptr, (const uint64_t *)d_b[1]->ptr, nullptr, nf, zd, wxf(), wyf(), xs, ys, bxf, byf,
+        (uint64_t *)w2->ptr, (uint64_t *)b2->ptr, stream()), "crc_conv2d_fold_pool");
+    chk(crc_stream_sync(ctx(), stream()), "crc_stream_sync");
+    d_w = w2; bxf = byf = 1;
 }
 bool MacLayer::limbFits() const
 {
@@ -938,10 +950,11 @@
         planned = plannedForm(B);
     }
     const bool conv1 = !dense && planned == CRC_NTTL1;
+    if (boxed() && !(conv1 && crc_limb_conv1_box_supported(ctx(), zd, xd, yd, xs, ys, wxf(), wyf(), nf, bxf, byf))) { unbox(); return limbWeights(B); }
     if (!conv1 && !(planned == CRC_NTTL && limbFits())) return false;
     if (w_form == CRC_NTTP) packWeights(true);
-    auto wl = make_shared<DeviceBuffer>(conv1 ? crc_limb_conv1_weights_bytes_for(ctx(), nf, xf, yf) : crc_limb_weights_bytes(ctx(), nf, zd, xf, yf));
-    if (conv1) chk(crc_limb_conv1_pack_weights(ctx(), (const uint64_t *)d_w->ptr, nf, xf, yf, wl->ptr, stream()), "crc_limb_conv1_pack_weights");
+    auto wl = make_shared<DeviceBuffer>(conv1 ? crc_limb_conv1_weights_bytes_for(ctx(), nf, wxf(), wyf()) : crc_limb_weights_bytes(ctx(), nf, zd, xf, yf));
+    if (conv1) chk(crc_limb_conv1_pack_weights(ctx(), (const uint64_t *)d_w->ptr, nf, wxf(), wyf(), wl->ptr, stream()), "crc_limb_conv1_pack_weights");
     else chk(crc_limb_pack_weights(ctx(), (const uint64_t *)d_w->ptr, nf, zd, xf, yf, wl->ptr, stream()), "crc_limb_pack_weights");
     chk(crc_stream_sync(ctx(), stream()), "crc_stream_sync");
     if (conv1) d_w_canon = d_w;
@@ -966,6 +979,16 @@
     last_B = input.B;
     ciphertext3D out(input.B, zo, xo, yo, out_form);
     if (streamed) { stream_form = forwardStreamed(input, out); return out; }
+    if (boxed() && w_form != CRC_NTTL1) unbox();
+    if (boxed()) {
+        const size_t bw = crc_conv2d_box_forms_work_bytes(ctx(), input.B, zd, xd, yd, xs, ys, wxf(), wyf(), nf, bxf, byf, input.form, w_form, out_form);
+        if (!bw) throw invalid_argument(kind() + string(": unsupported geometry"));
+        ensure(g_scratch, bw);
+        chk(crc_conv2d_box_forms(ctx(), input.data(), (const uint64_t *)d_w->ptr, w_form, (const uint64_t *)d_b[out_form != CRC_COEFF]->ptr, input.B, zd, xd, yd,
+            xs, ys, wxf(), wyf(), nf, bxf, byf, input.form, out_form, out.data(), g_scratch->ptr, stream()), "crc_conv2d_box_forms");
+        if (out_form == CRC_NTTLC) out.form = CRC_NTTL;
+        return out;
+    }
     size_t wb = crc_conv2d_forms_work_bytes(ctx(), input.B, zd, xd, yd, xs, ys, xf, yf, nf, input.form, w_form, out_form);
     if (!wb) throw invalid_argument(kind() + string(": unsupported geometry"));
     ensure(g_scratch, wb);
@@ -1652,6 +1675,12 @@
             g_expected_batch, matrix_cores ? 1 : 0, &hoist), "crc_plan_hoist_pool");
         if (hoist) {
             auto sums = foldPool(*up, up->name, 1, 1, pool->xf, pool->yf, nullptr);
+            int box = 0;
+            const bool bn_in_front = i >= 2 && !refreshBetween(i - 2) && dynamic_pointer_cast<BatchNormLayer>(layers[i - 2]);
+            if (!up->boxed() && !bn_in_front)
+                chk(crc_plan_conv1_box(ctx(), up->zd, up->xd, up->yd, up->xs, up->ys, up->xf, up->yf, up->nf, pool->xf, pool->yf, g_expected_batch,
+                    matrix_cores ? 1 : 0, &box), "crc_plan_conv1_box");
+            if (box) { sums->d_w = up->d_w; sums->bxf = pool->xf; sums->byf = pool->yf; }
             vector<Plaintext> nob; plaintext4D nof;
             auto down = make_shared<ConvolutionalLayer>(conv->name + "+" + pool->name, sums->xo, sums->yo, conv->zd, pool->xs, pool->ys, conv->xf, conv->yf,
                 conv->nf, conv->th_count, nof, nob);
@@ -1696,6 +1725,7 @@
         if (!bn || refreshBetween(i)) continue;
         auto m = dynamic_pointer_cast<MacLayer>(layers[i + 1]);
         if (!m) continue;
+        if (m->boxed()) { m->upload(); m->unbox(); }
         const int ch = bn->num_channels, T = (int)m->taps();
         if (m->dense ? T % ch != 0 : m->zd != ch) continue;
         const int per_ch = T / ch;
diff --git a/crcnn_amd/host/crcnn_host.h b/crcnn_amd/host/crcnn_host.h
--- a/crcnn_amd/host/crcnn_host.h
+++ b/crcnn_amd/host/crcnn_host.h
@@ -127,6 +127,7 @@
     void restoreCanonical();
     size_t deviceBytes() const override;
     std::string kernelName() const override;
+    void boxSize(int &bx, int &by) const { bx = bxf; by = byf; }
 protected:
     MacLayer(std::string name, bool dense, int zd, int xd, int yd, int xs, int ys, int xf, int yf, int nf)
         : Layer(name), zd(zd), xd(xd), yd(yd), xs(xs), ys(ys), xf(xf), yf(yf), nf(nf), dense(dense), slot_weights(slotEncoding()) {}
@@ -137,7 +138,12 @@
     virtual void plaintexts(int f0, int fn, std::vector<const Plaintext *> &w, std::vector<const Plaintext *> *b) const = 0;
     const bool dense;
     const char *kind() const { return dense ? "FullyConnectedLayer" : "ConvolutionalLayer"; }
-    size_t taps() const { return (size_t)zd * xf * yf; }
+    int bxf = 1, byf = 1;
+    bool boxed() const { return bxf * byf > 1; }
+    int wxf() const { return xf - (bxf - 1) * xs; }
+    int wyf() const { return yf - (byf - 1) * ys; }
+    void unbox();
+    size_t taps() const { return (size_t)zd * wxf() * wyf(); }
     std::shared_ptr<DeviceBuffer> d_w, d_b[2];
     bool streamed = false;
     int stream_form = CRC_NTT;
diff --git a/crcnn_amd/netrun.py b/crcnn_amd/netrun.py
--- a/crcnn_amd/netrun.py
+++ b/crcnn_amd/netrun.py
@@ -358,6 +358,11 @@
     def _geom(kind, a):
         return (a["zd"], a["xd"], a["yd"], a["xs"], a["ys"], a["xf"], a["yf"], a["nf"]) if kind == "conv" else (a["in_dim"], 1, 1, 1, 1, 1, 1, a["out_dim"])
 
+    @staticmethod
+    def _run_geom(a, p):
+        bxf, byf = p.get("box") or (1, 1)
+        return dict(a, xd=a["xd"] - (bxf - 1) * a["xs"], yd=a["yd"] - (byf - 1) * a["ys"], xf=a["xf"] - (bxf - 1) * a["xs"], yf=a["yf"] - (byf - 1) * a["ys"])
+
     def planned_form(self, kind, a, B=0):
         if kind not in ("conv", "fc"):
             return NTT
@@ -439,12 +444,13 @@
         assert not self._packed
         self._build_tilewise()
         for idx, (kind, name, a, p, ishape, oshape) in enumerate(self.plan):
-            if self.conv1_eligible(kind, a) and not p.get("streamed"):
-                nbytes = E.limb_conv1_weights_bytes_for(a["nf"], a["xf"], a["yf"])
+            ar = self._run_geom(a, p) if kind == "conv" else a
+            if self.conv1_eligible(kind, ar) and not p.get("streamed"):
+                nbytes = E.limb_conv1_weights_bytes_for(a["nf"], ar["xf"], ar["yf"])
                 wl = self.alloc(nbytes)
-                E.limb_conv1_pack_weights(p["w"], a["nf"], a["xf"], a["yf"], wl)
+                E.limb_conv1_pack_weights(p["w"], a["nf"], ar["xf"], ar["yf"], wl)
                 E.sync()
-                self.weight_bytes += nbytes - a["nf"] * a["xf"] * a["yf"] * E.k * E.n * 8
+                self.weight_bytes += nbytes - a["nf"] * ar["xf"] * ar["yf"] * E.k * E.n * 8
                 self._free(p["w"])
                 p["w"], p["w_form"] = wl, binding.NTTL1
                 continue
@@ -498,7 +504,8 @@
             if kind not in ("conv", "fc"):
                 continue
             if p.get("w_form") not in (binding.NTTL, binding.NTTL1) and not p.get("streamed"):
-                rows = (a["nf"] * a["zd"] * a["xf"] * a["yf"] if kind == "conv" else a["in_dim"] * a["out_dim"]) * E.k
+                ar = self._run_geom(a, p) if kind == "conv" else a
+                rows = (a["nf"] * a["zd"] * ar["xf"] * ar["yf"] if kind == "conv" else a["in_dim"] * a["out_dim"]) * E.k
                 E.pack28(p["w"], rows, unpack=unpack)
                 p["w_form"] = NTT if unpack else binding.NTTP
             nxt = self.plan[idx + 1] if idx + 1 < len(self.plan) else None
@@ -529,7 +536,10 @@
                 if same_shape and E.plan_fold_pool(a["zd"], a["xd"], a["yd"], a["xs"], a["ys"], a["xf"], a["yf"], a["nf"], pa["xs"], pa["ys"], pa["xf"], pa["yf"]):
                     up = plan[-1] if plan and plan[-1][0] == "conv" and not plan[-1][3].get("streamed") and not plan[-1][3].get("tilewise") and plan[-1][3]["out_form"] == NTT else None
                     if E.plan_hoist_pool(self._geom("conv", up[2]) if up else None, self._geom("conv", a), (pa["xs"], pa["ys"], pa["xf"], pa["yf"]), 0, matrix_cores=self.limb):
-                        plan[-1] = self._fold_sum_pool(up, pa["xf"], pa["yf"])
+                        ua = up[2]
+                        box = (not up[3].get("box") and not (len(plan) >= 2 and plan[-2][0] == "bn") and os.environ.get("CRC_MFMA_CONV1", "1") != "0"
+                               and E.plan_conv1_box(ua["zd"], ua["xd"], ua["yd"], ua["xs"], ua["ys"], ua["xf"], ua["yf"], ua["nf"], pa["xf"], pa["yf"], 0, matrix_cores=self.limb))
+                        plan[-1] = self._fold_sum_pool(up, pa["xf"], pa["yf"], box=box)
                         sshape = plan[-1][5]
                         cnt = a["nf"] * a["zd"] * a["xf"] * a["yf"]
                         w2 = self.alloc(cnt * E.k * E.n * 8); b2 = self.alloc(a["nf"] * E.k * E.n * 8)
@@ -563,7 +573,7 @@
         self._pair_square_pool()
         self._fold_batchnorm()
 
-    def _fold_sum_pool(self, entry, pxf, pyf):
+    def _fold_sum_pool(self, entry, pxf, pyf, box=False):
         E = self.E
         kind, name, a, p, ishape, oshape = entry
         xf2, yf2 = (pxf - 1) * a["xs"] + a["xf"], (pyf - 1) * a["ys"] + a["yf"]
@@ -572,10 +582,15 @@
         if self.materialize:
             E.conv2d_fold_pool(p["w"], p["b"], None, a["nf"], a["zd"], a["xf"], a["yf"], a["xs"], a["ys"], pxf, pyf, w2, b2)
             E.sync()
+        a2 = dict(a, xf=xf2, yf=yf2)
+        if box:
+            self.param_bufs = [(b_, n_) for (b_, n_) in self.param_bufs if b_ is not p["b"]] + [(b2, a["nf"] * E.k * E.n * 8)]
+            self._free(w2)
+            p2 = dict(p, b=b2, box=(pxf, pyf), macs=layer_macs("conv", a2))
+            return (kind, name, a2, p2, ishape, (oshape[0], oshape[1] - pxf + 1, oshape[2] - pyf + 1))
         self.param_bufs = [(b_, n_) for (b_, n_) in self.param_bufs if b_ is not p["w"] and b_ is not p["b"]]
         self.param_bufs += [(w2, cnt * E.k * E.n * 8), (b2, a["nf"] * E.k * E.n * 8)]
         self.weight_bytes += (cnt - a["nf"] * a["zd"] * a["xf"] * a["yf"]) * E.k * E.n * 8
-        a2 = dict(a, xf=xf2, yf=yf2)
         p2 = dict(p, w=w2, b=b2, macs=layer_macs("conv", a2))
         return (kind, name, a2, p2, ishape, (oshape[0], oshape[1] - pxf + 1, oshape[2] - pyf + 1))
 
@@ -619,7 +634,8 @@
         while i < len(self.plan):
             kind, name, a, p, ishape, oshape = self.plan[i]
             nxt = self.plan[i + 1] if i + 1 < len(self.plan) else None
-            if kind == "bn" and nxt and nxt[0] in ("conv", "fc") and p["form"] == NTT and nxt[3]["out_form"] == NTT and "fused" not in nxt[3] and not nxt[3].get("streamed"):
+            if (kind == "bn" and nxt and nxt[0] in ("conv", "fc") and p["form"] == NTT and nxt[3]["out_form"] == NTT and "fused" not in nxt[3] and not nxt[3].get("streamed")
+                    and not nxt[3].get("box")):
                 nk, nname, na, np_, nish, nosh = nxt
                 ch = ishape[0]
                 if nk == "conv":
@@ -736,7 +752,11 @@
                 else:
                     work = max(work, E.conv2d_forms_work_bytes(B, g["zd"], g["xd"], g["yd"], g["xs"], g["ys"], g["xf"], g["yf"], g["ft"], p["in_form"], NTT, p["out_form"]))
                 continue
-            if kind == "conv":
+            if kind == "conv" and p.get("box"):
+                ar = self._run_geom(a, p)
+                work = max(work, E.conv2d_box_forms_work_bytes(B, a["zd"], a["xd"], a["yd"], a["xs"], a["ys"], ar["xf"], ar["yf"], a["nf"], *p["box"], p["in_form"],
+                                                               p.get("w_form", NTT), p["out_form"]))
+            elif kind == "conv":
                 work = max(work, E.conv2d_forms_work_bytes(B, a["zd"], a["xd"], a["yd"], a["xs"], a["ys"], a["xf"], a["yf"], a["nf"], p["in_form"], p.get("w_form", NTT), p["out_form"]))
             elif kind == "fc":
                 work = max(work, E.conv2d_forms_work_bytes(B, a["in_dim"], 1, 1, 1, 1, 1, 1, a["out_dim"], p["in_form"], p.get("w_form", NTT), p["out_form"]))
@@ -907,6 +927,11 @@
             if p.get("streamed"):
                 self._forward_streamed(kind, a, p, cur, B, out)
                 cur = out
+            elif kind == "conv" and p.get("box"):
+                ar = self._run_geom(a, p)
+                E.conv2d_box(cur, p["w"], p["b"], B, a["zd"], a["xd"], a["yd"], a["xs"], a["ys"], ar["xf"], ar["yf"], a["nf"], *p["box"], p["in_form"], p["out_form"], out,
+                             self.work, w_form=p.get("w_form", NTT))
+                cur = out
             elif kind == "conv":
                 E.conv2d(cur, p["w"], p["b"], B, a["zd"], a["xd"], a["yd"], a["xs"], a["ys"], a["xf"], a["yf"], a["nf"], p["in_form"], p["out_form"], out, self.work,
                          w_form=p.get("w_form", NTT))
diff --git a/include/crcnn_hip.h b/include/crcnn_hip.h
--- a/include/crcnn_hip.h
+++ b/include/crcnn_hip.h
@@ -111,6 +111,12 @@
 int    crc_plan_fold_pool(const crc_ctx *ctx, int zd, int xd, int yd, int xs, int ys, int xf, int yf, int nf, int pxs, int pys, int pxf, int pyf, int *fold);
 int    crc_plan_hoist_pool(const crc_ctx *ctx, int uzd, int uxd, int uyd, int uxs, int uys, int uxf, int uyf, int unf, int zd, int xd, int yd, int xs, int ys,
                            int xf, int yf, int nf, int pxs, int pys, int pxf, int pyf, int B, int matrix_cores, int *hoist);
+int    crc_limb_conv1_box_supported(const crc_ctx *ctx, int zd, int xd, int yd, int xs, int ys, int xf, int yf, int nf, int bxf, int byf);
+size_t crc_conv2d_box_forms_work_bytes(const crc_ctx *ctx, int B, int zd, int xd, int yd, int xs, int ys, int xf, int yf, int nf, int bxf, int byf, int in_form,
+                                       int w_form, int out_form);
+int    crc_conv2d_box_forms(crc_ctx *ctx, const uint64_t *d_x, const uint64_t *d_w, int w_form, const uint64_t *d_bias_delta, int B, int zd, int xd, int yd,
+                            int xs, int ys, int xf, int yf, int nf, int bxf, int byf, int in_form, int out_form, uint64_t *d_y, void *d_work, void *stream);
+int    crc_plan_conv1_box(const crc_ctx *ctx, int zd, int xd, int yd, int xs, int ys, int xf, int yf, int nf, int bxf, int byf, int B, int matrix_cores, int *box);
 int    crc_limb_pack_tensor(crc_ctx *ctx, const uint64_t *d_x, int in_form, int B, int zd, int xd, int yd, void *d_xl, void *stream);
 int    crc_limb_pack_tensor_at(crc_ctx *ctx, const uint64_t *d_x, int in_form, int B, int zd, int xd, int yd, void *d_xl, int Btot, int b0, void *stream);
 int    crc_limb_conv1_supported(const crc_ctx *ctx, int zd, int xd, int yd, int xs, int ys, int xf, int yf, int nf);
```

Result: faster. 822.8, median of 6 (+2.9%).
